# helloybz/CLANE

Hardware: AMD Instinct MI355X
Metric: embedding-update iters/sec (Jacobi sweeps of Z <- X + gamma*P*Z, P frozen) (higher is better)
Workload: dtype f32; 1 GPU; R-MAT |V|=2000000 |E|=40000000 d=256 f32, gamma=0.76, CosineSimilarity (reference mode), seeds 3/4

## Files before the change

clane_amd/_hip.py:

```python
from __future__ import annotations

import abc
import ctypes as C
import os
import threading
from pathlib import Path
from typing import Optional

import torch

LIB_NAME = "libclane_hip.so"
LIB_PATH = Path(__file__).resolve().parent / LIB_NAME
ABI_VERSION = 5

SCORE_REFERENCE, SCORE_PER_EDGE, SCORE_RAW_DOT = 0, 1, 2
SPMM_SINKS_UNTOUCHED = 1
SPMM_TABLE_BEYOND_CACHE = 2
SCORE_FUSE_SOFTMAX = 1
SCORE_MODES = {"reference": SCORE_REFERENCE, "per_edge": SCORE_PER_EDGE, "raw_dot": SCORE_RAW_DOT}

_p, _i64, _i32 = C.c_void_p, C.c_int64, C.c_int32

SIGNATURES = {
    "clane_abi_version": (C.c_int, []),
    "clane_last_error": (C.c_char_p, []),
    "clane_build_info": (C.c_char_p, []),
    "clane_xcc_ids": (C.c_int, [_p, _i64, _i32, _p]),
    "clane_check_csr": (C.c_int, [_p, _p, _i64, _i64, _i64, _p, _p]),
    "clane_spmm_partials_len": (_i64, [_i64, _i64]),
    "clane_reduce_ws_len": (_i64, []),
    "clane_reduce_partials": (C.c_int, [_p, _i64, _p, _p, _p]),
    "clane_spmm_split_slab_len": (_i64, [_i64, _i32]),
    "clane_spmm_class_slab_len": (_i64, [_i64, _i32]),
    "clane_device_alloc": (C.c_int, [_i64, C.POINTER(_p)]),
    "clane_device_alloc_contiguous": (C.c_int, [_i64, C.POINTER(_p)]),
    "clane_device_free": (C.c_int, [_p]),
    "clane_ipc_export": (C.c_int, [_p, _p]),
    "clane_ipc_open": (C.c_int, [_p, C.POINTER(_p)]),
    "clane_ipc_close": (C.c_int, [_p]),
}
IPC_HANDLE_BYTES = 64
for _s in ("f32", "f64", "bf16"):
    SIGNATURES[f"clane_row_sqnorm_{_s}"] = (C.c_int, [_p, _i64, _i32, _i64, _p, _p])
    SIGNATURES[f"clane_edge_score_{_s}"] = (
        C.c_int, [_p, _p, _i64, _i64, _p, _i64, _i32, _i32, _p, _p, _p, _i32, _i64, _p, _i64, _p])
    _g = C.c_double if _s == "f64" else C.c_float
    SIGNATURES[f"clane_spmm_update_{_s}"] = (
        C.c_int, [_p, _p, _p, _i64, _i64, _p, _i64, _p, _i64, _g, _p, _i64, _i32, _i64, _i32, _p, _p, _p])
    SIGNATURES[f"clane_spmm_update_long_{_s}"] = (
        C.c_int, [_p, _p, _p, _p, _i64, _i32, _i64, _p, _i64, _p, _i64, _g, _p, _i64, _i32, _p, _p, _p])
    SIGNATURES[f"clane_spmm_update_split_{_s}"] = (
        C.c_int,
        [_p, _p, _p, _p, _p, _p, _i64, _i64, _i64, _i64, _p, _i64, _p, _i64, _g, _p, _i64, _i32, _p, _p, _p, _p])
    SIGNATURES[f"clane_spmm_update_class_{_s}"] = (
        C.c_int,
        [_p, _p, _p, _p, _p, _i64, _i32, _p, _p, _i64, _i64, _p, _i64, _p, _i64, _g, _p, _i64, _i32, _i32, _p, _p, _p, _p])
    SIGNATURES[f"clane_edge_score_class_{_s}"] = (
        C.c_int, [_p, _p, _p, _p, _p, _p, _i64, _i32, _p, _p, _i64, _i64, _p, _i64, _i32, _i32, _p, _p, _p, _i32, _p, _p])
    SIGNATURES[f"clane_gather_rows_{_s}"] = (C.c_int, [_p, _i64, _p, _i64, _i32, _p, _i64, _p])
    SIGNATURES[f"clane_l1_distance_{_s}"] = (C.c_int, [_p, _i64, _p, _i64, _i64, _i32, _p, _p, _p, _p])
SIGNATURES["clane_spmm_update_owned_f32"] = (
    C.c_int, [_p, _p, _p, _i32, _i64, _p, _i64, _p, _i64, C.c_float, _p, _i64, _i32, _i32, _p, _p])
for _s in ("f32", "f64"):
    SIGNATURES[f"clane_degree_weighted_sums_{_s}"] = (C.c_int, [_p, _p, _p, _i64, _p, _p, _p])
    SIGNATURES[f"clane_edge_score_finalize_{_s}"] = (C.c_int, [_p, _p, _i64, _i64, _i32, _p, _p, _p, _p])
    SIGNATURES[f"clane_segment_softmax_{_s}"] = (C.c_int, [_p, _i64, _p, _i64, _i64, _p, _i64, _p])
    SIGNATURES[f"clane_pair_cosine_{_s}"] = (C.c_int, [_p, _i64, _p, _i64, _i64, _i32, _p, _p, _p])
    SIGNATURES[f"clane_edge_score_pair_{_s}"] = (
        C.c_int, [_p, _p, _i64, _i64, _p, _i64, _p, _i64, _i32, _p, _i32, _i64, _p, _i64, _p])
    SIGNATURES[f"clane_edge_score_class_pair_{_s}"] = (
        C.c_int, [_p, _p, _p, _p, _p, _p, _i64, _i32, _p, _p, _i64, _i64, _p, _i64, _p, _i64, _i32, _p, _i32, _p, _p])
for _s in ("f32", "f64", "bf16"):
    SIGNATURES[f"clane_project_rows_{_s}"] = (C.c_int, [_p, _i64, _i32, _i64, _p, _p, _i64, _p])
    SIGNATURES[f"clane_pair_project_{_s}"] = (C.c_int, [_p, _i64, _i32, _i64, _p, _p, _i64, _p, _p, _p, _p])
    SIGNATURES[f"clane_pair_grad_{_s}"] = (C.c_int, [_p, _i64, _i32, _i64, _p, _p, _i64, _p, _p, _p, _p, _p, _p, _p])
for _s in ("f32", "f64"):
    SIGNATURES[f"clane_pair_loss_{_s}"] = (C.c_int, [_p, _p, _i64, _i32, _p, _p, _p, _p, _p, _p, _p])
    SIGNATURES[f"clane_adam_step_{_s}"] = (C.c_int, [_p, _p, _p, _p, _i64, C.c_double, _p, _p, _p])
SIGNATURES["clane_pair_grad_ws_len"] = (_i64, [_i64, _i32])
RANK_MAX_K = 32
for _s in ("f32", "f64", "bf16"):
    SIGNATURES[f"clane_rank_scores_{_s}"] = (
        C.c_int, [_p, _i64, _p, _i64, _i64, _i32, _p, _i64, _i32, _p, _p, _p, _p, _p, _i32, _i32, _i32, _p, _p, _p])
    SIGNATURES[f"clane_pair_score_{_s}"] = (C.c_int, [_p, _i64, _p, _i64, _i64, _i32, _p, _p, _i64, _i32, _p, _p, _p, _p])
    SIGNATURES[f"clane_rank_count_{_s}"] = (
        C.c_int, [_p, _i64, _p, _i64, _i64, _i32, _p, _p, _i64, _i32, _p, _p, _p, _p, _p, _i32, _i32, _p, _p, _p])
for _s in ("f32", "f64"):
    SIGNATURES[f"clane_rank_merge_{_s}"] = (C.c_int, [_p, _p, _i64, _i32, _i32, _p, _p, _p])
SIGNATURES["clane_pair_labels"] = (C.c_int, [_p, _p, _i64, _p, _p, _i64, _p, _p])
PROBE_MAX_CLASSES = 64
PROBE_WRITE_G, PROBE_WRITE_PRED = 1, 2
PROBE_PRED_TOPK = 4
for _s in ("f32", "f64", "bf16"):
    SIGNATURES[f"clane_probe_forward_{_s}"] = (
        C.c_int, [_p, _i64, _i32, _i64, _p, _p, _i64, _p, _i64, _p, _p, _i32, _i32, _i32, _p, _p, _p, _p, _i64, _p])
    SIGNATURES[f"clane_probe_grad_{_s}"] = (C.c_int, [_p, _i64, _i32, _i64, _p, _i64, _p, _i32, _p, _p, _p, _p])
    SIGNATURES[f"clane_probe_forward_ovr_{_s}"] = (
        C.c_int, [_p, _i64, _i32, _i64, _p, _p, _i64, _p, _i64, _p, _p, _p, _i32, _i32, _i32, _i32, _p, _p, _p, _p, _i64, _p])
SIGNATURES["clane_probe_loss_ws_len"] = (_i64, [_i64, _i32])
SIGNATURES["clane_probe_grad_ws_len"] = (_i64, [_i64, _i32, _i32])
for _s in ("f32", "f64", "bf16"):
    SIGNATURES[f"clane_kmeans_assign_{_s}"] = (
        C.c_int, [_p, _i64, _i32, _i64, _p, _i64, _p, _p, _i32, _i32, _p, _i64, _p, _i64, _p])
    SIGNATURES[f"clane_kmeans_update_{_s}"] = (
        C.c_int, [_p, _i64, _i32, _i64, _p, _p, _i64, _i32, _i32, _p, _p, _p, _p, _p])
SIGNATURES["clane_kmeans_update_ws_len"] = (_i64, [_i64, _i32, _i32, _i32])
for _s in ("f32", "f64", "bf16"):
    _g = C.c_double if _s == "f64" else C.c_float
    SIGNATURES[f"clane_embed_rows_{_s}"] = (
        C.c_int, [_p, _p, _i64, _p, _i64, _p, _i64, _i64, _i32, _i32, _p, _p, _p, _i64, _g, _i32, _i32, _i32, _p, _i64,
                  _p, _p, _p, _p])

PCA_ACCUMULATE = 1
for _s in ("f32", "f64", "bf16"):
    SIGNATURES[f"clane_column_sums_{_s}"] = (C.c_int, [_p, _i64, _i32, _i64, _p, _i64, _i32, _p, _p, _p])
# ... 345 lines not shown
    def probe_forward_ovr(self, Z, d: int, rows, ymask, split, W, bias, col_state, F: int, C: int, max_labels: int,
                          loss_ws, loss, G=None, pred=None, top_k: bool = True):
        raise NotImplementedError(f"{type(self).__name__} has no probe_forward_ovr")

    def probe_grad_ws_len(self, n: int, K: int, d: int) -> int:
        raise NotImplementedError(f"{type(self).__name__} has no probe_grad_ws_len")

    def probe_grad(self, Z, d: int, rows, G, ws, dW, db):
        raise NotImplementedError(f"{type(self).__name__} has no probe_grad")

    def kmeans_assign(self, Z, d: int, rows, centres, csq, assign, best):
        raise NotImplementedError(f"{type(self).__name__} has no kmeans_assign")

    def kmeans_update_ws_len(self, n: int, R: int, K: int, d: int) -> int:
        raise NotImplementedError(f"{type(self).__name__} has no kmeans_update_ws_len")

    def kmeans_update(self, Z, d: int, order, seg, centres_old, ws, centres_new, csq_new):
        raise NotImplementedError(f"{type(self).__name__} has no kmeans_update")

    def column_sums_ws_len(self, n: int, d: int) -> int:
        raise NotImplementedError(f"{type(self).__name__} has no column_sums_ws_len")

    def column_sums(self, Z, d: int, rows, ws, sums, accumulate: bool = False):
        raise NotImplementedError(f"{type(self).__name__} has no column_sums")

    def gram_ws_len(self, n: int, d: int) -> int:
        raise NotImplementedError(f"{type(self).__name__} has no gram_ws_len")

    def gram(self, Z, d: int, rows, mu, ws, G, accumulate: bool = False):
        raise NotImplementedError(f"{type(self).__name__} has no gram")

    def project_affine(self, Z, d: int, rows, mu, W, Y):
        raise NotImplementedError(f"{type(self).__name__} has no project_affine")

    def csr_spmm_segment(self) -> int:
        raise NotImplementedError(f"{type(self).__name__} has no csr_spmm_segment")

    def csr_spmm_ws_len(self, n_rows: int, nnz: int, l: int) -> int:
        raise NotImplementedError(f"{type(self).__name__} has no csr_spmm_ws_len")

    def csr_spmm(self, S, B, l: int, out, a=None, s=None, ws=None):
        raise NotImplementedError(f"{type(self).__name__} has no csr_spmm")

    def csr_row_sums(self, S, sums, ws=None):
        raise NotImplementedError(f"{type(self).__name__} has no csr_row_sums")

    def has_spmm_owned(self, dtype, d: int) -> bool:
        return False

    def make_owned_plan(self, plan: dict, chunk: int, device):
        raise NotImplementedError(f"{type(self).__name__} has no make_owned_plan")

    def spmm_update_owned(self, colidx, P, plan, block_threads: int, row0: int, Z_old, X, gamma: float, Z_new, d: int,
                          partials, beyond_cache: bool = False, loads: int = 0):
        raise NotImplementedError(f"{type(self).__name__} has no spmm_update_owned")

    def bind(self, method: str, *args, **kwargs):
        fn = getattr(self, method)
        return lambda: fn(*args, **kwargs)

    def embed_rows(self, rowptr, colidx, X_new, Z, table_rows: int, d: int, mode: int, sums2, sq, S, gamma: float,
                   tolerence: int, max_rounds: int, Z_out, rounds, delta, P_out=None, flags: int = 0):
        raise NotImplementedError(f"{type(self).__name__} has no embed_rows")


class HipKernels(KernelBackend):

    def __init__(self, lib: Optional[C.CDLL] = None):
        self.lib = lib if lib is not None else load_library()
        self._tls = threading.local()

    def _invoke(self, fn, what: str, *cargs):
        rec = getattr(self._tls, "recording", None)
        if rec is not None:
            rec.append((fn, cargs, what))
        else:
            self._check(fn(*cargs), what)

    def bind(self, method: str, *args, **kwargs):
        self._tls.recording = []
        try:
            getattr(self, method)(*args, **kwargs)
            (fn, cargs, what), = self._tls.recording
        finally:
            self._tls.recording = None
        check = self._check
        return lambda: check(fn(*cargs), what)

    def _check(self, rc: int, what: str):
        if rc != 0:
            raise ClaneHipError(f"{what} failed ({rc}): {self.lib.clane_last_error().decode()}")

    @staticmethod
    def _stream(t: torch.Tensor):
        if not t.is_cuda:
            raise ClaneHipError("HipKernels needs tensors in GPU memory (got a CPU tensor); there is no CPU path")
        return torch.cuda.current_stream(t.device).cuda_stream

    def _fn(self, base: str, dtype: torch.dtype):
        try:
            return getattr(self.lib, f"{base}_{_SUFFIX[dtype]}")
        except KeyError:
            raise TypeError(f"{base}: unsupported dtype {dtype}") from None

    def spmm_partials_len(self, nrows: int, n_long: int) -> int:
        return int(self.lib.clane_spmm_partials_len(nrows, n_long))

    def xcc_ids(self, n_blocks: int, block_threads: int = 256, device=None) -> torch.Tensor:
        out = torch.full((n_blocks,), -1, dtype=torch.int32, device=device if device is not None else "cuda")
        self._check(self.lib.clane_xcc_ids(out.data_ptr(), n_blocks, block_threads, self._stream(out)), "clane_xcc_ids")
        return out

    def check_csr(self, rowptr: torch.Tensor, colidx: torch.Tensor, nrows: int, n_edges: int, table_rows: int) -> None:
        if rowptr.dtype != torch.int64 or colidx.dtype != torch.int32 or rowptr.numel() < nrows + 1 or colidx.numel() < n_edges:
            raise ValueError("check_csr: rowptr must be int64 [nrows + 1], colidx int32 [n_edges]")
        status = torch.zeros(1, dtype=torch.int32, device=rowptr.device)
        self._check(self.lib.clane_check_csr(rowptr.data_ptr(), colidx.data_ptr(), nrows, n_edges, table_rows,
                                             status.data_ptr(), self._stream(rowptr)), "clane_check_csr")
        bad = int(status.item())
# ... 100 lines not shown
        if not (Z_old.dtype == X.dtype == Z_new.dtype):
            raise ValueError("spmm_update_long: Z_old, X, Z_new must share a dtype")
        self._invoke(self._fn("clane_spmm_update_long", Z_old.dtype), "clane_spmm_update_long",
                     _vec(rowptr, torch.int64, "rowptr"), _vec(colidx, torch.int32, "colidx"),
                     _vec(P, acc_dtype(Z_old.dtype), "P"), _vec(long_rows, torch.int32, "long_rows"),
                     long_rows.numel(), waves_per_row, row0, zo, ldz, xp, ldx, gamma, zn, ldo, d,
                     _mirror_arg(mirror, Z_new.dtype), _vec(partials, torch.float64, "partials"), self._stream(Z_old))

    def spmm_split_slab_len(self, n_segments: int, d: int) -> int:
        return int(self.lib.clane_spmm_split_slab_len(n_segments, d))

    def spmm_update_split(self, rowptr, colidx, P, split_rows, seg_ptr, seg_row, edges_per_segment: int, row0: int,
                          Z_old, X, gamma: float, Z_new, d: int, slab, partials, mirror: Optional[Mirror] = None):
        zo, ldz = _mat(Z_old, "Z_old")
        xp, ldx = _mat(X, "X")
        zn, ldo = _mat(Z_new, "Z_new")
        self._invoke(self._fn("clane_spmm_update_split", Z_old.dtype), "clane_spmm_update_split",
                     _vec(rowptr, torch.int64, "rowptr"), _vec(colidx, torch.int32, "colidx"),
                     _vec(P, acc_dtype(Z_old.dtype), "P"), _vec(split_rows, torch.int32, "split_rows"),
                     _vec(seg_ptr, torch.int64, "seg_ptr"), _vec(seg_row, torch.int32, "seg_row"),
                     split_rows.numel(), seg_row.numel(), edges_per_segment, row0, zo, ldz, xp, ldx, gamma, zn, ldo, d,
                     _vec(slab, acc_dtype(Z_old.dtype), "slab"), _mirror_arg(mirror, Z_new.dtype),
                     _vec(partials, torch.float64, "partials"), self._stream(Z_old))

    def spmm_class_slab_len(self, n_slots: int, d: int) -> int:
        return int(self.lib.clane_spmm_class_slab_len(n_slots, d))

    def spmm_update_class(self, colidx, P, item_e0, item_len, item_slot, items_per_block: int, class_rows, slot_ptr,
                          row0: int, Z_old, X, gamma: float, Z_new, d: int, slab, partials,
                          mirror: Optional[Mirror] = None, beyond_cache: bool = False):
        zo, ldz = _mat(Z_old, "Z_old")
        xp, ldx = _mat(X, "X")
        zn, ldo = _mat(Z_new, "Z_new")
        n_items = item_e0.numel()
        if n_items % items_per_block or item_len.numel() != n_items or item_slot.numel() != n_items:
            raise ValueError("spmm_update_class: the item arrays must hold whole blocks of items_per_block items")
        self._invoke(self._fn("clane_spmm_update_class", Z_old.dtype), "clane_spmm_update_class",
                     _vec(colidx, torch.int32, "colidx"), _vec(P, acc_dtype(Z_old.dtype), "P"),
                     _vec(item_e0, torch.int64, "item_e0"), _vec(item_len, torch.int32, "item_len"),
                     _vec(item_slot, torch.int32, "item_slot"), n_items // items_per_block, items_per_block,
                     _vec(class_rows, torch.int32, "class_rows"), _vec(slot_ptr, torch.int64, "slot_ptr"),
                     class_rows.numel(), row0, zo, ldz, xp, ldx, gamma, zn, ldo, d,
                     SPMM_TABLE_BEYOND_CACHE if beyond_cache else 0,
                     _vec(slab, acc_dtype(Z_old.dtype), "slab"), _mirror_arg(mirror, Z_new.dtype),
                     _vec(partials, torch.float64, "partials"), self._stream(Z_old))

    def has_spmm_owned(self, dtype, d: int) -> bool:
        return dtype == torch.float32 and 64 < d <= 256

    def make_owned_plan(self, plan: dict, chunk: int, device) -> OwnedPlan:
        return OwnedPlan(plan, chunk, device)

    def spmm_update_owned(self, colidx, P, plan: OwnedPlan, block_threads: int, row0: int, Z_old, X, gamma: float,
                          Z_new, d: int, partials, beyond_cache: bool = False, loads: int = 0):
        zo, ldz = _mat(Z_old, "Z_old")
        xp, ldx = _mat(X, "X")
        zn, ldo = _mat(Z_new, "Z_new")
        if not (Z_old.dtype == X.dtype == Z_new.dtype == torch.float32):
            raise TypeError("spmm_update_owned: float32 tables only")
        lanes = 32 if d <= 128 else 64
        if plan.max_batch_vrows * lanes * 16 > OWNED_LDS_LIMIT:
            raise ValueError(f"spmm_update_owned: {plan.max_batch_vrows} virtual rows per batch do not fit the LDS")
        if (plan.max_edge > min(colidx.numel(), P.numel()) or plan.max_row >= min(X.shape[0], Z_new.shape[0])
                or row0 + plan.max_row >= Z_old.shape[0] or plan.max_part >= partials.numel()):
            raise ValueError("spmm_update_owned: the plan reaches outside colidx / P, the tables or the partials")
        self._invoke(self.lib.clane_spmm_update_owned_f32, "clane_spmm_update_owned",
                     _vec(colidx, torch.int32, "colidx"), _vec(P, torch.float32, "P"), C.cast(C.pointer(plan.c), _p),
                     int(block_threads), row0, zo, ldz, xp, ldx, gamma, zn, ldo, d,
                     (SPMM_TABLE_BEYOND_CACHE if beyond_cache else 0) | ((int(loads) & 0xff) << 8),
                     _vec(partials, torch.float64, "partials"), self._stream(Z_old))

    def reduce_partials(self, partials, n: int, ws, out):
        self._invoke(self.lib.clane_reduce_partials, "clane_reduce_partials",
                     _vec(partials, torch.float64, "partials"), n, _vec(ws, torch.float64, "ws"),
                     _vec(out, torch.float64, "out"), self._stream(out))

    def l1_distance(self, A, B, d: int, ws, out, sq_a: Optional[torch.Tensor] = None):
        ap, lda = _mat(A, "A")
        bp, ldb = _mat(B, "B")
        self._check(self._fn("clane_l1_distance", A.dtype)(
            ap, lda, bp, ldb, A.shape[0], d, self._sq_arg(sq_a, A.dtype), _vec(ws, torch.float64, "ws"),
            _vec(out, torch.float64, "out"), self._stream(A)), "clane_l1_distance")

    def gather_rows(self, src, idx, d: int, dst):
        sp, lds = _mat(src, "src")
        dp, ldd = _mat(dst, "dst")
        self._invoke(self._fn("clane_gather_rows", src.dtype), "clane_gather_rows",
                     sp, lds, _vec(idx, torch.int32, "idx"), idx.numel(), d, dp, ldd, self._stream(src))

    def project_rows(self, Z, d: int, W, Y):
        zp, ldz = _mat(Z, "Z")
        yp, ldy = _mat(Y, "Y")
        acc = acc_dtype(Z.dtype)
        if tuple(W.shape) != (2 * d, d):
            raise ValueError(f"project_rows: W must be [2d, d] = [{2 * d}, {d}], got {tuple(W.shape)}")
        if Y.dtype != acc or Y.shape[0] < Z.shape[0]:
            raise ValueError(f"project_rows: Y must be {acc} with at least {Z.shape[0]} rows")
        self._check(self._fn("clane_project_rows", Z.dtype)(
            zp, Z.shape[0], d, ldz, _vec(W, acc, "W"), yp, ldy, self._stream(Z)), "clane_project_rows")

    def edge_score_pair(self, rowptr, colidx, nrows: int, row0: int, S, N, d: int, scores, long_threshold: int = 0,
                        long_rows=None, fuse_softmax: bool = False):
        sp, lds = _mat(S, "S")
        np_, ldn = _mat(N, "N")
        if S.dtype != N.dtype:
            raise ValueError("edge_score_pair: S and N must share a dtype")
        n_long = 0 if long_rows is None else long_rows.numel()
        self._check(self._fn("clane_edge_score_pair", S.dtype)(
            _vec(rowptr, torch.int64, "rowptr"), _vec(colidx, torch.int32, "colidx"), nrows, row0, sp, lds, np_, ldn, d,
            _vec(scores, S.dtype, "scores"), SCORE_FUSE_SOFTMAX if fuse_softmax else 0, long_threshold,
            None if n_long == 0 else _vec(long_rows, torch.int32, "long_rows"), n_long,
            self._stream(S)), "clane_edge_score_pair")

    def edge_score_class_pair(self, rowptr, colidx, item_e0, item_len, item_slot, item_row, items_per_block: int,
                              class_rows, slot_ptr, row0: int, S, N, d: int, scores, stats=None,
                              fuse_softmax: bool = False, n_slots: Optional[int] = None, row_parts: int = 1):
        sp, lds = _mat(S, "S")
        np_, ldn = _mat(N, "N")
        if S.dtype != N.dtype:
            raise ValueError("edge_score_class_pair: S and N must share a dtype")
        n_items = item_e0.numel()
        if n_items % items_per_block or any(t.numel() != n_items for t in (item_len, item_slot, item_row)):
            raise ValueError("edge_score_class_pair: the item arrays must hold whole blocks of items_per_block items")
# ... 406 lines not shown
```

clane_amd/csrc/clane_abi.hip:

```cpp
#include "../../include/clane_hip.h"

#include <hip/hip_runtime.h>

#include <climits>
#include <cstdarg>
#include <cstdio>
#include <cstring>

#include "build_p.h"
#include "content_pca.h"
#include "edge_score.h"
#include "device_utils.h"
#include "kmeans.h"
#include "label_probe.h"
#include "multilabel_probe.h"
#include "new_rows.h"
#include "link_eval.h"
#include "link_rank.h"
#include "pair_train.h"
#include "projection.h"
#include "sparse_rows.h"
#include "spmm_update.h"

namespace {
// ... 428 lines not shown
        spmm_class_combine_kernel<T, VEC, LPR>
            <<<unsigned(ceil_div(n_split, kWave / LPR)), kCombineWaves * kWave, 0, (hipStream_t)stream>>>(
            split_rows, seg_ptr, n_split, row0, slab, ld_slab, Z_old, ldz, X, ldx, gamma, Z_new, ldo, d, mir, false, delta_partials);
    });
    return check_launch("spmm_update_split");
}

template <typename T, typename PT>
int spmm_update_class(const int32_t *colidx, const PT *P, const int64_t *item_e0, const int32_t *item_len,
                      const int32_t *item_slot, int64_t n_blocks, int32_t items_per_block, const int32_t *class_rows,
                      const int64_t *slot_ptr, int64_t n_rows, int64_t row0, const T *Z_old, int64_t ldz, const T *X,
                      int64_t ldx, typename Elem<T>::acc_t gamma, T *Z_new, int64_t ldo, int32_t d, int32_t flags,
                      typename Elem<T>::acc_t *slab, const clane_mirror_t *mirror, double *delta_partials,
                      void *stream) {
    REQUIRE(mirror_ok(mirror, d), "spmm_update_class: incomplete mirror descriptor");
    REQUIRE(n_blocks >= 0 && n_blocks <= INT32_MAX && n_rows >= 0 && n_rows <= INT32_MAX && row0 >= 0 && d > 0,
            "spmm_update_class: bad shape");
    REQUIRE(items_per_block >= kWavesPerBlock && items_per_block <= kMaxItemsPerBlock,
            "spmm_update_class: items_per_block must be in [%d, %d]", kWavesPerBlock, kMaxItemsPerBlock);
    REQUIRE(ldz >= d && ldx >= d && ldo >= d, "spmm_update_class: leading dimension < d");
    if (n_rows == 0) return CLANE_OK;
    REQUIRE(colidx && P && item_e0 && item_len && item_slot && class_rows && slot_ptr && Z_old && X && Z_new && slab &&
                delta_partials,
            "spmm_update_class: null pointer");
    REQUIRE((const void *)Z_new != (const void *)Z_old, "spmm_update_class: Z_new must not alias Z_old");
    REQUIRE(aligned16(slab), "spmm_update_class: slab must be 16-byte aligned");
    const Layout L = pick_layout<T>(d, {Z_old, X, Z_new, mirror_alignment_probe(mirror, Z_new)},
                                    {ldz, ldx, ldo, mirror && mirror->row_ptr ? mirror->ld : ldo});
    const int64_t ld_slab = ceil_div(d, 8) * 8;
    const Mirror<T> mir = make_mirror<T>(mirror);
    dispatch_layout<T>(L, [&]<int VEC, int LPR>() {
        constexpr int U = VEC > 1 ? CLANE_LONG_U : 4;
        constexpr int kDeepU = (LPR == 32 && VEC == 4 && sizeof(T) == 4) ? CLANE_CLASS_U32
                               : (LPR == 16 && VEC == 8 && sizeof(T) == 2) ? CLANE_CLASS_U16B : 0;
        if (n_blocks > 0 && kDeepU > 0 && (flags & CLANE_SPMM_TABLE_BEYOND_CACHE))
            spmm_class_chunk_kernel<T, PT, VEC, LPR, (kDeepU > 0 ? kDeepU : U)>
                <<<unsigned(n_blocks), kBlock, 0, (hipStream_t)stream>>>(
                    colidx, P, item_e0, item_len, item_slot, items_per_block, Z_old, ldz, d, slab, ld_slab);
        else if (n_blocks > 0)
            spmm_class_chunk_kernel<T, PT, VEC, LPR, U><<<unsigned(n_blocks), kBlock, 0, (hipStream_t)stream>>>(
                colidx, P, item_e0, item_len, item_slot, items_per_block, Z_old, ldz, d, slab, ld_slab);
        spmm_class_combine_kernel<T, VEC, LPR>
            <<<unsigned(ceil_div(n_rows, kWave / LPR)), kCombineWaves * kWave, 0, (hipStream_t)stream>>>(
            class_rows, slot_ptr, n_rows, row0, slab, ld_slab, Z_old, ldz, X, ldx, gamma, Z_new, ldo, d, mir,
            (flags & CLANE_SPMM_TABLE_BEYOND_CACHE) != 0, delta_partials);
    });
    return check_launch("spmm_update_class");
}

constexpr int64_t kOwnedLdsReserve = 1024;
constexpr int64_t kLdsPerCU = 160 * 1024;
constexpr int64_t kLdsDefaultLimit = 64 * 1024;

template <typename T, typename PT>
int spmm_update_owned(const int32_t *colidx, const PT *P, const clane_owned_plan_t *plan, int32_t block_threads,
                      int64_t row0, const T *Z_old, int64_t ldz, const T *X, int64_t ldx,
                      typename Elem<T>::acc_t gamma, T *Z_new, int64_t ldo, int32_t d, int32_t flags,
                      double *delta_partials, void *stream) {
    using A = typename Elem<T>::acc_t;
    REQUIRE(plan, "spmm_update_owned: null plan");
    REQUIRE(plan->n_groups >= 0 && row0 >= 0 && d > 0, "spmm_update_owned: bad shape");
    REQUIRE(plan->n_steps >= 1 && plan->n_steps <= kOwnedMaxSteps, "spmm_update_owned: n_steps must be in [1, %d]",
            kOwnedMaxSteps);
    REQUIRE(plan->chunk >= kWave && plan->chunk % kWave == 0, "spmm_update_owned: chunk must be a positive multiple of 64");
    REQUIRE(block_threads >= kWave && block_threads <= kOwnedMaxBlock && block_threads % kWave == 0,
            "spmm_update_owned: block_threads must be a multiple of 64 in [64, %d]", kOwnedMaxBlock);
    REQUIRE(ldz >= d && ldx >= d && ldo >= d, "spmm_update_owned: leading dimension < d");
    REQUIRE(plan->max_batch_vrows >= 0, "spmm_update_owned: negative max_batch_vrows");
    if (plan->n_groups == 0) return CLANE_OK;
    REQUIRE(colidx && P && plan->grp_bat_ptr && plan->bat_vrow_ptr && plan->bat_row_ptr && plan->bat_seg_ptr &&
                plan->seg_e0 && plan->seg_len && plan->seg_vrow && plan->row_id && plan->row_part && plan->row_vptr &&
                Z_old && X && Z_new && delta_partials,
            "spmm_update_owned: null pointer");
    REQUIRE((const void *)Z_new != (const void *)Z_old, "spmm_update_owned: Z_new must not alias Z_old");
    const Layout L = pick_layout<T>(d, {Z_old, X, Z_new}, {ldz, ldx, ldo});
    REQUIRE(L.vec && (L.lpr == 32 || L.lpr == 64) && d <= L.lpr * Elem<T>::kVec,
            "spmm_update_owned: no instance for d=%d with these operands (16-byte packs, 17..64 packs per row)", d);
    const int64_t lds = int64_t(plan->max_batch_vrows) * L.lpr * Elem<T>::kVec * int64_t(sizeof(A));
    REQUIRE(lds + kOwnedLdsReserve <= kLdsPerCU, "spmm_update_owned: %lld virtual rows per batch need %lld bytes of LDS",
            (long long)plan->max_batch_vrows, (long long)lds);
    const OwnedPlan op{plan->grp_bat_ptr, plan->bat_vrow_ptr, plan->bat_row_ptr, plan->bat_seg_ptr, plan->seg_e0,
                       plan->seg_len, plan->seg_vrow, plan->row_id, plan->row_part, plan->row_vptr, plan->n_steps,
                       plan->chunk};
    const bool beyond = (flags & CLANE_SPMM_TABLE_BEYOND_CACHE) != 0;
    int rc = CLANE_OK;
    auto launch = [&]<int VEC, int LPR, int U>() {
        auto *kernel = spmm_owned_kernel<T, PT, VEC, LPR, U>;
        if (lds > kLdsDefaultLimit) {
            static int64_t granted = 0;
            if (lds > granted) {
                const hipError_t e = hipFuncSetAttribute(reinterpret_cast<const void *>(kernel),
                                                         hipFuncAttributeMaxDynamicSharedMemorySize, int(lds));
                if (e != hipSuccess) {
                    rc = fail(CLANE_ERR_LAUNCH, "spmm_update_owned: %lld bytes of LDS: %s", (long long)lds,
                              hipGetErrorString(e));
                    return;
                }
                granted = lds;
            }
        }
        kernel<<<unsigned(plan->n_groups), unsigned(block_threads), size_t(lds), (hipStream_t)stream>>>(
            colidx, P, op, row0, Z_old, ldz, X, ldx, gamma, Z_new, ldo, d, beyond, delta_partials);
    };
    constexpr int KV = Elem<T>::kVec;
    const int asked = (flags >> 8) & 0xff;
    REQUIRE(asked == 0 || asked == 8 || asked == 12 || (L.lpr == 32 && asked == 6),
            "spmm_update_owned: no instance with %d row loads in flight", asked);
    const int loads = asked ? asked : (L.lpr == 32 && beyond) ? CLANE_CLASS_U32 : CLANE_LONG_U;
    if (L.lpr == 32) {
        if (loads == 6) launch.template operator()<KV, 32, 6>();
        else if (loads == 12) launch.template operator()<KV, 32, 12>();
        else launch.template operator()<KV, 32, 8>();
    } else {
        if (loads == 12) launch.template operator()<KV, 64, 12>();
        else launch.template operator()<KV, 64, 8>();
    }
    if (rc != CLANE_OK) return rc;
    return check_launch("spmm_update_owned");
}

template <typename T>
int l1_distance(const T *A, int64_t lda, const T *B, int64_t ldb, int64_t nrows, int32_t d,
                typename Elem<T>::acc_t *sq_a, double *ws, double *out, void *stream) {
    REQUIRE(nrows >= 0 && d > 0 && lda >= d && ldb >= d, "l1_distance: bad shape");
    REQUIRE(ws && out, "l1_distance: null workspace/output");
    REQUIRE(nrows == 0 || (A && B), "l1_distance: null pointer");
    const Layout L = pick_layout<T>(d, {A, B}, {lda, ldb});
    if (sq_a != nullptr) {
        const Layout LA = pick_layout<T>(d, {A}, {lda});
        REQUIRE(LA.vec == L.vec && LA.lpr == L.lpr,
                "l1_distance: sq_a needs B as aligned as A (the lane layout of row_sqnorm on A)");
    }
    int grid = 1;
    dispatch_layout<T>(L, [&]<int VEC, int LPR>() {
        grid = grid_for_waves(ceil_div(nrows > 0 ? nrows : 1, (kWave / LPR) * stream_rows(LPR)));
        if (grid > kReduceGrid) grid = kReduceGrid;
        l1_distance_kernel<T, VEC, LPR><<<grid, kBlock, 0, (hipStream_t)stream>>>(A, lda, B, ldb, nrows, d, sq_a, ws);
    });
    reduce_fixed_kernel<<<1, 1024, 0, (hipStream_t)stream>>>(ws, grid, grid, 1, out);
    return check_launch("l1_distance");
}

template <typename T>
int gather_rows(const T *src, int64_t lds, const int32_t *idx, int64_t n, int32_t d, T *dst, int64_t ldd, void *stream) {
    REQUIRE(n >= 0 && d > 0 && lds >= d && ldd >= d, "gather_rows: bad shape");
    if (n == 0) return CLANE_OK;
    REQUIRE(src && idx && dst, "gather_rows: null pointer");
    const Layout L = pick_layout<T>(d, {src, dst}, {lds, ldd});
    dispatch_layout<T>(L, [&]<int VEC, int LPR>() {
        const int grid = grid_for_waves(ceil_div(n, kWave / LPR));
        gather_rows_kernel<T, VEC, LPR><<<grid, kBlock, 0, (hipStream_t)stream>>>(src, lds, idx, n, d, dst, ldd);
    });
    return check_launch("gather_rows");
}

template <typename T>
int pair_cosine(const T *A, int64_t lda, const T *B, int64_t ldb, int64_t nrows, int32_t d,
                typename Elem<T>::acc_t *out, double *ws, void *stream) {
    REQUIRE(nrows >= 0 && d > 0 && lda >= d && ldb >= d, "pair_cosine: bad shape");
    if (nrows == 0) return CLANE_OK;
    REQUIRE(A && B && out && ws, "pair_cosine: null pointer");
    const Layout L = pick_layout<T>(d, {A, B}, {lda, ldb});
    int grid = 1;
    dispatch_layout<T>(L, [&]<int VEC, int LPR>() {
        grid = grid_for_waves(ceil_div(nrows, kWave / LPR));
        if (grid > kReduceGrid) grid = kReduceGrid;
        pair_dot_kernel<T, VEC, LPR><<<grid, kBlock, 0, (hipStream_t)stream>>>(A, lda, B, ldb, nrows, d, out, ws);
    });
    double *sums2 = ws + 2 * kReduceGrid;
    reduce_fixed_kernel<<<1, 1024, 0, (hipStream_t)stream>>>(ws, grid, grid, 2, sums2);
    int sgrid = int(ceil_div(nrows, kBlock));
// ... 688 lines not shown
                                CT *Z_new, int64_t ldo, int32_t d, int64_t long_threshold, int32_t flags,             \
                                const clane_mirror_t *mirror, double *delta_partials, void *stream) {                \
        return spmm_update<T, PT>(rowptr, colidx, P, nrows, row0, reinterpret_cast<const T *>(Z_old), ldz,            \
                                  reinterpret_cast<const T *>(X), ldx, gamma, reinterpret_cast<T *>(Z_new), ldo, d,   \
                                  long_threshold, flags, mirror, delta_partials, stream);                             \
    }                                                                                                                 \
    int clane_spmm_update_long_##SUF(const int64_t *rowptr, const int32_t *colidx, const PT *P,                       \
                                     const int32_t *long_rows, int64_t n_long, int32_t waves_per_row, int64_t row0, const CT *Z_old,         \
                                     int64_t ldz, const CT *X, int64_t ldx, GT gamma, CT *Z_new, int64_t ldo,         \
                                     int32_t d, const clane_mirror_t *mirror, double *delta_partials, void *stream) { \
        return spmm_update_long<T, PT>(rowptr, colidx, P, long_rows, n_long, waves_per_row, row0,                     \
                                       reinterpret_cast<const T *>(Z_old), ldz, reinterpret_cast<const T *>(X), ldx,  \
                                       gamma, reinterpret_cast<T *>(Z_new), ldo, d, mirror, delta_partials, stream);  \
    }
#define CLANE_SPLIT_WRAPPER(SUF, CT, T, PT, GT)                                                                         \
    int clane_spmm_update_split_##SUF(const int64_t *rowptr, const int32_t *colidx, const PT *P,                      \
                                      const int32_t *split_rows, const int64_t *seg_ptr, const int32_t *seg_row,      \
                                      int64_t n_split, int64_t n_segments, int64_t edges_per_segment, int64_t row0,   \
                                      const CT *Z_old, int64_t ldz, const CT *X, int64_t ldx, GT gamma, CT *Z_new,    \
                                      int64_t ldo, int32_t d, GT *slab, const clane_mirror_t *mirror,                 \
                                      double *delta_partials, void *stream) {                                         \
        return spmm_update_split<T, PT>(rowptr, colidx, P, split_rows, seg_ptr, seg_row, n_split, n_segments,         \
                                        edges_per_segment, row0, reinterpret_cast<const T *>(Z_old), ldz,             \
                                        reinterpret_cast<const T *>(X), ldx, gamma, reinterpret_cast<T *>(Z_new),     \
                                        ldo, d, slab, mirror, delta_partials, stream);                                \
    }
CLANE_SPLIT_WRAPPER(f32, float, float, float, float)
CLANE_SPLIT_WRAPPER(f64, double, double, double, double)
CLANE_SPLIT_WRAPPER(bf16, uint16_t, bf16_t, float, float)
#undef CLANE_SPLIT_WRAPPER
#define CLANE_CLASS_WRAPPER(SUF, CT, T, PT, GT)                                                                        \
    int clane_spmm_update_class_##SUF(const int32_t *colidx, const PT *P, const int64_t *item_e0,                     \
                                      const int32_t *item_len, const int32_t *item_slot, int64_t n_blocks,            \
                                      int32_t items_per_block, const int32_t *class_rows, const int64_t *slot_ptr,    \
                                      int64_t n_rows, int64_t row0, const CT *Z_old, int64_t ldz, const CT *X,        \
                                      int64_t ldx, GT gamma, CT *Z_new, int64_t ldo, int32_t d, int32_t flags,        \
                                      GT *slab, const clane_mirror_t *mirror, double *delta_partials, void *stream) { \
        return spmm_update_class<T, PT>(colidx, P, item_e0, item_len, item_slot, n_blocks, items_per_block,           \
                                        class_rows, slot_ptr, n_rows, row0, reinterpret_cast<const T *>(Z_old), ldz,  \
                                        reinterpret_cast<const T *>(X), ldx, gamma, reinterpret_cast<T *>(Z_new),     \
                                        ldo, d, flags, slab, mirror, delta_partials, stream);                         \
    }
CLANE_CLASS_WRAPPER(f32, float, float, float, float)
CLANE_CLASS_WRAPPER(f64, double, double, double, double)
CLANE_CLASS_WRAPPER(bf16, uint16_t, bf16_t, float, float)
#undef CLANE_CLASS_WRAPPER
int clane_spmm_update_owned_f32(const int32_t *colidx, const float *P, const clane_owned_plan_t *plan,
                                int32_t block_threads, int64_t row0, const float *Z_old, int64_t ldz, const float *X,
                                int64_t ldx, float gamma, float *Z_new, int64_t ldo, int32_t d, int32_t flags,
                                double *delta_partials, void *stream) {
    return spmm_update_owned<float, float>(colidx, P, plan, block_threads, row0, Z_old, ldz, X, ldx, gamma, Z_new, ldo,
                                           d, flags, delta_partials, stream);
}
int64_t clane_spmm_class_slab_len(int64_t n_slots, int32_t d) { return n_slots * (ceil_div(d, 8) * 8); }
int64_t clane_spmm_split_slab_len(int64_t n_segments, int32_t d) { return n_segments * (ceil_div(d, 8) * 8); }

CLANE_SPMM_WRAPPERS(f32, float, float, float, float)
CLANE_SPMM_WRAPPERS(f64, double, double, double, double)
CLANE_SPMM_WRAPPERS(bf16, uint16_t, bf16_t, float, float)
#undef CLANE_SPMM_WRAPPERS

int clane_reduce_partials(const double *partials, int64_t n, double *ws, double *out, void *stream) {
    if (n < 0 || !out || !ws || (n > 0 && !partials))
        return fail(CLANE_ERR_INVALID_ARGUMENT, "reduce_partials: bad arguments");
    if (n <= 8192) {
        reduce_fixed_kernel<<<1, 1024, 0, (hipStream_t)stream>>>(partials, n, n, 1, out);
    } else {
        const int64_t slice = ceil_div(n, kReduceGrid);
        const int grid = int(ceil_div(n, slice));
        reduce_slices_kernel<<<grid, kBlock, 0, (hipStream_t)stream>>>(partials, n, slice, ws);
        reduce_fixed_kernel<<<1, 1024, 0, (hipStream_t)stream>>>(ws, grid, grid, 1, out);
    }
    return check_launch("reduce_partials");
}

int clane_l1_distance_f32(const float *A, int64_t lda, const float *B, int64_t ldb, int64_t nrows, int32_t d,
                          float *sq_a, double *ws, double *out, void *stream) {
    return l1_distance<float>(A, lda, B, ldb, nrows, d, sq_a, ws, out, stream);
}
int clane_l1_distance_f64(const double *A, int64_t lda, const double *B, int64_t ldb, int64_t nrows, int32_t d,
                          double *sq_a, double *ws, double *out, void *stream) {
    return l1_distance<double>(A, lda, B, ldb, nrows, d, sq_a, ws, out, stream);
}
int clane_l1_distance_bf16(const uint16_t *A, int64_t lda, const uint16_t *B, int64_t ldb, int64_t nrows, int32_t d,
                           float *sq_a, double *ws, double *out, void *stream) {
    return l1_distance<bf16_t>(reinterpret_cast<const bf16_t *>(A), lda, reinterpret_cast<const bf16_t *>(B), ldb,
                               nrows, d, sq_a, ws, out, stream);
}

int clane_gather_rows_f32(const float *src, int64_t lds, const int32_t *idx, int64_t n, int32_t d, float *dst,
                          int64_t ldd, void *stream) {
    return gather_rows<float>(src, lds, idx, n, d, dst, ldd, stream);
}
int clane_gather_rows_f64(const double *src, int64_t lds, const int32_t *idx, int64_t n, int32_t d, double *dst,
                          int64_t ldd, void *stream) {
    return gather_rows<double>(src, lds, idx, n, d, dst, ldd, stream);
}
int clane_gather_rows_bf16(const uint16_t *src, int64_t lds, const int32_t *idx, int64_t n, int32_t d, uint16_t *dst,
                           int64_t ldd, void *stream) {
    return gather_rows<bf16_t>(reinterpret_cast<const bf16_t *>(src), lds, idx, n, d,
                               reinterpret_cast<bf16_t *>(dst), ldd, stream);
}

int clane_pair_cosine_f32(const float *A, int64_t lda, const float *B, int64_t ldb, int64_t nrows, int32_t d,
                          float *out, double *ws, void *stream) {
    return pair_cosine<float>(A, lda, B, ldb, nrows, d, out, ws, stream);
// ... 197 lines not shown
```

clane_amd/csrc/spmm_update.h:

```cpp
#pragma once

#include "device_utils.h"

#ifndef CLANE_SPMM_U
#define CLANE_SPMM_U 8
#endif
#ifndef CLANE_SPMM_DYNAMIC
#define CLANE_SPMM_DYNAMIC 1
#endif
#ifndef CLANE_COMBINE_WAVES
#define CLANE_COMBINE_WAVES 2
#endif
#ifndef CLANE_SPMM_PREFETCH
#define CLANE_SPMM_PREFETCH 1
#endif
#ifndef CLANE_SPMM_MIN_WAVES
#define CLANE_SPMM_MIN_WAVES 0
#endif

namespace clane {

template <typename A>
struct EdgeChunk {
    int c;
// ... 114 lines not shown
    return rsum;
}

template <typename T, int VEC, int GROUP>
__device__ __forceinline__ void mirror_store(const Mirror<T> &mirror, int64_t row, int col, const Pack<T, VEC> &out,
                                             bool writer, int group_lane, int base) {
    if (mirror.row_ptr == nullptr) return;
    const int64_t s0 = mirror.row_ptr[row], s1 = mirror.row_ptr[row + 1];
    for (int64_t s = s0; s < s1; s += GROUP) {
        const int n = s1 - s < GROUP ? int(s1 - s) : GROUP;
        int32_t mine = 0;
        if (group_lane < n) mine = mirror.slot[s + group_lane];
        for (int j = 0; j < n; ++j) {
            int32_t place;
            if constexpr (GROUP == kWave) place = lane_get_uniform(mine, j);
            else place = lane_get(mine, base + j);
            if (writer) store_pack<T, VEC>(mirror.row(place) + col, out);
        }
    }
}

template <typename T, int VEC, int GROUP>
__device__ __forceinline__ void mirror_store_prefetched(const Mirror<T> &mirror, int64_t m0, int64_t m1, int32_t mine,
                                                        int col, const Pack<T, VEC> &out, bool writer, int group_lane,
                                                        int base) {
    if (mirror.row_ptr == nullptr) return;
    const int n = m1 - m0 < GROUP ? int(m1 - m0) : GROUP;
    for (int j = 0; j < n; ++j) {
        int32_t place;
        if constexpr (GROUP == kWave) place = lane_get_uniform(mine, j);
        else place = lane_get(mine, base + j);
        if (writer) store_pack<T, VEC>(mirror.row(place) + col, out);
    }
    for (int64_t s = m0 + GROUP; s < m1; s += GROUP) {
        const int k = m1 - s < GROUP ? int(m1 - s) : GROUP;
        int32_t more = 0;
        if (group_lane < k) more = mirror.slot[s + group_lane];
        for (int j = 0; j < k; ++j) {
            int32_t place;
            if constexpr (GROUP == kWave) place = lane_get_uniform(more, j);
            else place = lane_get(more, base + j);
            if (writer) store_pack<T, VEC>(mirror.row(place) + col, out);
        }
    }
}

#if CLANE_SPMM_MIN_WAVES > 0
#define CLANE_SPMM_BOUNDS __launch_bounds__(kBlock, CLANE_SPMM_MIN_WAVES)
#else
#define CLANE_SPMM_BOUNDS __launch_bounds__(kBlock)
#endif

template <typename T, typename PT, int VEC, int LPR, int U, bool MIRRORED>
__global__ CLANE_SPMM_BOUNDS void spmm_update_kernel(
    const int64_t *__restrict__ rowptr, const int32_t *__restrict__ colidx, const PT *__restrict__ P, int64_t nrows,
    int64_t row0, const T *__restrict__ Zold, int64_t ldz, const T *__restrict__ X, int64_t ldx,
    typename Elem<T>::acc_t gamma, T *__restrict__ Znew, int64_t ldo, int d, int64_t long_threshold,
    bool skip_sinks, int rows_per_block, Mirror<T> mirror, bool nt_store, double *__restrict__ partials) {
    using A = typename Elem<T>::acc_t;
    __shared__ int64_t s_rowptr[kMaxRowsPerBlock + 1];
    __shared__ int64_t s_mptr[MIRRORED ? kMaxRowsPerBlock + 1 : 1];
    __shared__ double s_rowsum[kMaxRowsPerBlock];
    __shared__ int s_next;
    __shared__ int s_done;

    const int lane = lane_id();
    const int wave = __builtin_amdgcn_readfirstlane(threadIdx.x / kWave);
    const int sub = lane / LPR;
    const int sl = lane % LPR;
    const int64_t row_begin = int64_t(blockIdx.x) * rows_per_block;
    const int nb = int((row_begin + rows_per_block < nrows ? row_begin + rows_per_block : nrows) - row_begin);

    for (int i = threadIdx.x; i <= nb; i += kBlock) {
        s_rowptr[i] = rowptr[row_begin + i];
        if constexpr (MIRRORED) s_mptr[i] = mirror.row_ptr[row_begin + i];
    }
    for (int i = threadIdx.x; i < nb; i += kBlock) s_rowsum[i] = 0.0;
    if (threadIdx.x == 0) {
        s_next = kWavesPerBlock;
        s_done = 0;
    }
    __syncthreads();
    auto places_of = [&]([[maybe_unused]] int row, [[maybe_unused]] int64_t &m0, [[maybe_unused]] int64_t &m1) -> int32_t {
        if constexpr (MIRRORED) {
            m0 = s_mptr[row];
            m1 = s_mptr[row + 1];
            return lane < m1 - m0 ? mirror.slot[m0 + lane] : 0;
        } else {
            return 0;
        }
    };

    auto claim = [&]([[maybe_unused]] int prev) -> int {
#if CLANE_SPMM_DYNAMIC
        int v = 0;
        if (lane == 0) v = atomicAdd(&s_next, 1);
        return __builtin_amdgcn_readfirstlane(v);
#else
        return prev + kWavesPerBlock;
#endif
    };

    int cur = wave;
    int64_t e0 = 0, e1 = 0, m0 = 0, m1 = 0;
    int32_t places = 0;
    EdgeChunk<A> ch{0, A(0)};
    if (cur < nb) {
        e0 = s_rowptr[cur];
        e1 = s_rowptr[cur + 1];
        ch = load_chunk<A, PT>(colidx, P, e0, e1);
        places = places_of(cur, m0, m1);
    }
    while (cur < nb) {
        const int nxt = claim(cur);
        int64_t n0 = 0, n1 = 0, mn0 = 0, mn1 = 0;
        int32_t places_n = 0;
        EdgeChunk<A> chn{0, A(0)};
        if (nxt < nb) {
            n0 = s_rowptr[nxt];
            n1 = s_rowptr[nxt + 1];
#if CLANE_SPMM_PREFETCH
            chn = load_chunk<A, PT>(colidx, P, n0, n1);
#endif
            places_n = places_of(nxt, mn0, mn1);
        }
        if (!(long_threshold > 0 && e1 - e0 > long_threshold) && !(skip_sinks && e1 == e0)) {
            const int64_t r = row_begin + cur;
            A rsum = A(0);
            for (int t0 = 0; t0 < d; t0 += LPR * VEC) {
                const int c0 = t0 + sl * VEC;
                const bool col_ok = c0 < d;
                const bool writer = col_ok && sub == 0;
                Pack<T, VEC> x{}, zo{};
                if (writer) {
                    x = load_pack_stream<T, VEC>(X + r * ldx + c0);
                    zo = load_pack_stream<T, VEC>(Zold + (row0 + r) * ldz + c0);
                }
                A acc[VEC];
#pragma unroll
                for (int k = 0; k < VEC; ++k) acc[k] = A(0);
                gather_accumulate<T, PT, VEC, LPR, U>(colidx, P, e0, e1, Zold + (col_ok ? c0 : 0), ldz, col_ok, acc, ch, true);
                fold_subwaves<LPR>(acc);
                Pack<T, VEC> out{};
                if (writer) rsum += finish_pack<T, VEC>(x, zo, acc, gamma, e1 > e0, Znew + r * ldo + c0, out, nt_store);
                if constexpr (MIRRORED)
                    mirror_store_prefetched<T, VEC, kWave>(mirror, m0, m1, places, c0, out, writer, lane, 0);
            }
            rsum = group_sum<kWave>(rsum);
            if (lane == 0) s_rowsum[cur] = double(rsum);
        }
        cur = nxt;
        e0 = n0;
        e1 = n1;
        m0 = mn0;
        m1 = mn1;
        places = places_n;
#if CLANE_SPMM_PREFETCH
        ch = chn;
#else
        if (cur < nb) ch = load_chunk<A, PT>(colidx, P, e0, e1);
#endif
    }
    if (!last_wave_of_block(&s_done)) return;
    double dsum = 0.0;
    for (int i = lane; i < nb; i += kWave) dsum += s_rowsum[i];
    dsum = group_sum<kWave>(dsum);
    if (lane == 0) partials[blockIdx.x] = dsum;
}

#ifndef CLANE_SUBROW_MIN_WAVES
#define CLANE_SUBROW_MIN_WAVES 0
#endif
#if CLANE_SUBROW_MIN_WAVES > 0
#define CLANE_SUBROW_BOUNDS __launch_bounds__(kBlock, (sizeof(typename Elem<T>::acc_t) == 8 ? 1 : CLANE_SUBROW_MIN_WAVES))
#else
#define CLANE_SUBROW_BOUNDS __launch_bounds__(kBlock)
#endif
template <typename T, typename PT, int VEC, int LPR, int U, bool MIRRORED>
__global__ CLANE_SUBROW_BOUNDS void spmm_update_subrow_kernel(
    const int64_t *__restrict__ rowptr, const int32_t *__restrict__ colidx, const PT *__restrict__ P, int64_t nrows,
    int64_t row0, const T *__restrict__ Zold, int64_t ldz, const T *__restrict__ X, int64_t ldx,
    typename Elem<T>::acc_t gamma, T *__restrict__ Znew, int64_t ldo, int d, int64_t long_threshold,
    bool skip_sinks, int rows_per_block, Mirror<T> mirror, bool nt_store, double *__restrict__ partials) {
    using A = typename Elem<T>::acc_t;
    static_assert(LPR < kWave, "use spmm_update_kernel for rows that fill a wave");
    static_assert(LPR % U == 0, "a sub-wave's edge buffer is consumed in whole groups of U");
    __shared__ int64_t s_rowptr[kMaxRowsPerBlock + 1];
    __shared__ int64_t s_mptr[MIRRORED ? kMaxRowsPerBlock + 1 : 1];
    __shared__ double s_rowsum[kMaxRowsPerBlock];
    __shared__ int s_next;
    __shared__ int s_done;

    const int lane = lane_id();
    const int sub = lane / LPR;
    const int sl = lane % LPR;
    const int sub_base = sub * LPR;
    const int64_t row_begin = int64_t(blockIdx.x) * rows_per_block;
    const int nb = int((row_begin + rows_per_block < nrows ? row_begin + rows_per_block : nrows) - row_begin);
    const int c0 = sl * VEC;
    const bool col_ok = c0 < d;
    const int c0s = col_ok ? c0 : 0;

    for (int i = threadIdx.x; i <= nb; i += kBlock) {
        s_rowptr[i] = rowptr[row_begin + i];
        if constexpr (MIRRORED) s_mptr[i] = mirror.row_ptr[row_begin + i];
    }
    for (int i = threadIdx.x; i < nb; i += kBlock) s_rowsum[i] = 0.0;
    if (threadIdx.x == 0) {
        s_next = 0;
        s_done = 0;
    }
    __syncthreads();

    int mine = 0;
    bool have = false;
    bool done = false;
    int64_t e_next = 0;
    int64_t e_end = 0;
    int nbuf = 0, pos = 0;
    int c = 0;
    A p = A(0);
    [[maybe_unused]] int64_t m0 = 0, m1 = 0;
    [[maybe_unused]] int32_t places = 0;
    Pack<T, VEC> x{}, zo{};
    A acc[VEC];
#pragma unroll
    for (int k = 0; k < VEC; ++k) acc[k] = A(0);

    for (;;) {
        if (pos >= nbuf && !done) {
            if (e_next == e_end) {
                if (have) {
                    const int64_t r = row_begin + mine;
                    A rsum = A(0);
                    Pack<T, VEC> out{};
                    if (col_ok) rsum = finish_pack<T, VEC>(x, zo, acc, gamma, true, Znew + r * ldo + c0, out, nt_store);
                    if constexpr (MIRRORED)
                        mirror_store_prefetched<T, VEC, LPR>(mirror, m0, m1, places, c0, out, col_ok, sl, sub_base);
                    rsum = group_sum<LPR>(rsum);
                    if (sl == 0) s_rowsum[mine] = double(rsum);
                    have = false;
                }
                for (;;) {
                    int v = 0;
                    if (sl == 0) v = atomicAdd(&s_next, 1);
                    mine = lane_get(v, sub_base);
                    if (mine >= nb) {
                        done = true;
                        break;
                    }
// ... 12 lines not shown
                        m0 = s_mptr[mine];
                        m1 = s_mptr[mine + 1];
                        places = sl < m1 - m0 ? mirror.slot[m0 + sl] : 0;
                    }
                    if (col_ok) {
                        x = load_pack_stream<T, VEC>(X + r * ldx + c0);
                        zo = load_pack_stream<T, VEC>(Zold + (row0 + r) * ldz + c0);
                    }
#pragma unroll
                    for (int k = 0; k < VEC; ++k) acc[k] = A(0);
                    have = true;
                    break;
                }
            }
            pos = 0;
            nbuf = 0;
            c = 0;
            p = A(0);
            if (!done) {
                const int64_t left = e_end - e_next;
                nbuf = left < LPR ? int(left) : LPR;
                if (sl < nbuf) {
                    c = colidx[e_next + sl];
                    p = A(P[e_next + sl]);
                }
                e_next += nbuf;
            }
        }
        if (__all(done)) break;
        Pack<T, VEC> z[U];
        A pj[U];
#pragma unroll
        for (int u = 0; u < U; ++u) {
            const int src = sub_base + ((pos + u) & (LPR - 1));
            const int cj = lane_get(c, src);
            pj[u] = lane_get(p, src);
            z[u] = load_pack<T, VEC>(Zold + int64_t(cj) * ldz + c0s);
        }
#pragma unroll
        for (int u = 0; u < U; ++u) {
#pragma unroll
            for (int k = 0; k < VEC; ++k) {
                A zv = Elem<T>::to_acc(z[u].v[k]);
                zv = pj[u] != A(0) ? zv : A(0);
                acc[k] = fma(pj[u], zv, acc[k]);
            }
        }
        pos += U;
    }
    if (!last_wave_of_block(&s_done)) return;
    double dsum = 0.0;
    for (int i = lane; i < nb; i += kWave) dsum += s_rowsum[i];
    dsum = group_sum<kWave>(dsum);
    if (lane == 0) partials[blockIdx.x] = dsum;
}

template <typename T, typename PT, int VEC, int LPR, int U, int WAVES>
__global__ __launch_bounds__(WAVES *kWave) void spmm_long_kernel(
    const int64_t *__restrict__ rowptr, const int32_t *__restrict__ colidx, const PT *__restrict__ P,
    const int32_t *__restrict__ long_rows, int64_t row0, const T *__restrict__ Zold, int64_t ldz,
    const T *__restrict__ X, int64_t ldx, typename Elem<T>::acc_t gamma, T *__restrict__ Znew, int64_t ldo, int d,
    Mirror<T> mirror, double *__restrict__ partials) {
    using A = typename Elem<T>::acc_t;
    __shared__ A red[WAVES][kWave][VEC];
    const int lane = lane_id();
    const int wave = __builtin_amdgcn_readfirstlane(threadIdx.x / kWave);
    const int sub = lane / LPR;
    const int sl = lane % LPR;
    const int64_t r = long_rows[blockIdx.x];
    const int64_t e0 = rowptr[r];
    const int64_t e1 = rowptr[r + 1];
    const int64_t seg = ceil_div(ceil_div(e1 - e0, WAVES), kWave) * kWave;
    const int active = e1 > e0 ? int(ceil_div(e1 - e0, seg)) : 1;
    if (idle_wave_may_exit(wave < active)) return;
    const int64_t a = e0 + wave * seg;
    const int64_t b = a + seg < e1 ? a + seg : e1;
    const EdgeChunk<A> none{0, A(0)};
    A rsum = A(0);

    for (int t0 = 0; t0 < d; t0 += LPR * VEC) {
        const int c0 = t0 + sl * VEC;
        const bool col_ok = c0 < d;
        const bool writer = wave == 0 && col_ok && sub == 0;
        Pack<T, VEC> x{}, zo{};
        if (writer) {
            x = load_pack_stream<T, VEC>(X + r * ldx + c0);
            zo = load_pack_stream<T, VEC>(Zold + (row0 + r) * ldz + c0);
        }
        A acc[VEC];
#pragma unroll
        for (int k = 0; k < VEC; ++k) acc[k] = A(0);
        gather_accumulate<T, PT, VEC, LPR, U>(colidx, P, a, b, Zold + (col_ok ? c0 : 0), ldz, col_ok, acc, none, false);
        fold_subwaves<LPR>(acc);
        if (wave > 0) {
#pragma unroll
            for (int k = 0; k < VEC; ++k) red[wave][lane][k] = acc[k];
        }
        __syncthreads();
        if (wave == 0) {
            Pack<T, VEC> out{};
            if (writer) {
                for (int w = 1; w < active; ++w) {
#pragma unroll
                    for (int k = 0; k < VEC; ++k) acc[k] += red[w][lane][k];
                }
                rsum += finish_pack<T, VEC>(x, zo, acc, gamma, e1 > e0, Znew + r * ldo + c0, out, false);
            }
// ... 42 lines not shown
        for (int k = 0; k < VEC; ++k) acc[k] = A(0);
        gather_accumulate<T, PT, VEC, LPR, U>(colidx, P, a, b, Zold + (col_ok ? c0 : 0), ldz, col_ok, acc, none, false);
        fold_subwaves<LPR>(acc);
        if (wave > 0) {
#pragma unroll
            for (int k = 0; k < VEC; ++k) red[wave][lane][k] = acc[k];
        }
        __syncthreads();
        if (wave == 0 && col_ok && sub == 0) {
            for (int w = 1; w < active; ++w) {
#pragma unroll
                for (int k = 0; k < VEC; ++k) acc[k] += red[w][lane][k];
            }
            Pack<A, VEC> o;
#pragma unroll
            for (int k = 0; k < VEC; ++k) o.v[k] = acc[k];
            store_pack<A, VEC>(slab + s * ld_slab + c0, o);
        }
        if (t0 + LPR * VEC < d) __syncthreads();
    }
}

}

namespace clane {


#ifndef CLANE_NT_SLAB
#define CLANE_NT_SLAB 1
#endif
template <typename A, int VEC>
__device__ __forceinline__ void slab_store(A *p, const Pack<A, VEC> &v) {
    if constexpr ((CLANE_NT_SLAB & 1) && sizeof(Pack<A, VEC>) == 16) {
        clane_u32x4 w;
        __builtin_memcpy(&w, &v, 16);
        __builtin_nontemporal_store(w, reinterpret_cast<clane_u32x4 *>(p));
    } else {
        store_pack<A, VEC>(p, v);
    }
}
template <typename A, int VEC>
__device__ __forceinline__ Pack<A, VEC> slab_load(const A *p) {
    if constexpr ((CLANE_NT_SLAB & 2) && sizeof(Pack<A, VEC>) == 16) {
        const clane_u32x4 v = __builtin_nontemporal_load(reinterpret_cast<const clane_u32x4 *>(p));
        Pack<A, VEC> out;
        __builtin_memcpy(&out, &v, 16);
        return out;
    } else {
        return load_pack<A, VEC>(p);
    }
}

template <typename T, typename PT, int VEC, int LPR, int U>
__global__ __launch_bounds__(kBlock) void spmm_class_chunk_kernel(
    const int32_t *__restrict__ colidx, const PT *__restrict__ P, const int64_t *__restrict__ item_e0,
    const int32_t *__restrict__ item_len, const int32_t *__restrict__ item_slot, int items_per_block,
    const T *__restrict__ Zold, int64_t ldz, int d, typename Elem<T>::acc_t *__restrict__ slab, int64_t ld_slab) {
    using A = typename Elem<T>::acc_t;
    __shared__ int64_t s_e0[kMaxItemsPerBlock];
    __shared__ int s_len[kMaxItemsPerBlock];
    __shared__ int s_slot[kMaxItemsPerBlock];
    __shared__ int s_next;
    const int lane = lane_id();
    const int wave = __builtin_amdgcn_readfirstlane(threadIdx.x / kWave);
    const int sub = lane / LPR;
    const int sl = lane % LPR;
    const int64_t base = int64_t(blockIdx.x) * items_per_block;
    for (int i = threadIdx.x; i < items_per_block; i += kBlock) {
        s_e0[i] = item_e0[base + i];
        s_len[i] = item_len[base + i];
        s_slot[i] = item_slot[base + i];
    }
    if (threadIdx.x == 0) s_next = kWavesPerBlock;
    __syncthreads();

    auto claim = [&]() -> int {
        int v = 0;
        if (lane == 0) v = atomicAdd(&s_next, 1);
        return __builtin_amdgcn_readfirstlane(v);
    };
    int cur = wave;
    int64_t e0 = 0, e1 = 0;
    EdgeChunk<A> ch{0, A(0)};
    if (cur < items_per_block) {
        e0 = s_e0[cur];
        e1 = e0 + s_len[cur];
        ch = load_chunk<A, PT>(colidx, P, e0, e1);
    }
    while (cur < items_per_block) {
        const int nxt = claim();
        int64_t n0 = 0, n1 = 0;
        EdgeChunk<A> chn{0, A(0)};
        if (nxt < items_per_block) {
            n0 = s_e0[nxt];
            n1 = n0 + s_len[nxt];
            chn = load_chunk<A, PT>(colidx, P, n0, n1);
        }
        if (e1 > e0) {
            A *out = slab + int64_t(s_slot[cur]) * ld_slab;
            for (int t0 = 0; t0 < d; t0 += LPR * VEC) {
                const int c0 = t0 + sl * VEC;
                const bool col_ok = c0 < d;
                A acc[VEC];
#pragma unroll
                for (int k = 0; k < VEC; ++k) acc[k] = A(0);
                gather_accumulate<T, PT, VEC, LPR, U>(colidx, P, e0, e1, Zold + (col_ok ? c0 : 0), ldz, col_ok, acc, ch, true);
                fold_subwaves<LPR>(acc);
                if (col_ok && sub == 0) {
                    Pack<A, VEC> o;
#pragma unroll
                    for (int k = 0; k < VEC; ++k) o.v[k] = acc[k];
                    slab_store<A, VEC>(out + c0, o);
                }
            }
        }
        cur = nxt;
        e0 = n0;
        e1 = n1;
        ch = chn;
    }
}

constexpr int kCombineWaves = CLANE_COMBINE_WAVES;
#ifndef CLANE_COMBINE_LOADS
#define CLANE_COMBINE_LOADS 16
#endif
constexpr int kCombineLoads = CLANE_COMBINE_LOADS;

template <typename T, int VEC, int LPR>
__global__ __launch_bounds__(kCombineWaves *kWave) void spmm_class_combine_kernel(
    const int32_t *__restrict__ class_rows, const int64_t *__restrict__ slot_ptr, int64_t n_rows, int64_t row0,
    const typename Elem<T>::acc_t *__restrict__ slab, int64_t ld_slab, const T *__restrict__ Zold, int64_t ldz,
    const T *__restrict__ X, int64_t ldx, typename Elem<T>::acc_t gamma, T *__restrict__ Znew, int64_t ldo, int d,
    Mirror<T> mirror, bool nt_store, double *__restrict__ partials) {
    using A = typename Elem<T>::acc_t;
    constexpr int kRows = kWave / LPR;
    __shared__ A s_part[kCombineWaves > 1 ? kCombineWaves - 1 : 1][kWave][VEC];
    const int lane = lane_id();
    const int wave = __builtin_amdgcn_readfirstlane(threadIdx.x / kWave);
    const int sub = lane / LPR, sl = lane % LPR;
    const int64_t i = int64_t(blockIdx.x) * kRows + sub;
    const bool live = i < n_rows;
    const int64_t r = live ? class_rows[i] : 0;
    const int64_t s0 = live ? slot_ptr[i] : 0, s1 = live ? slot_ptr[i + 1] : 0;
    const int64_t share = ceil_div(s1 - s0, int64_t(kCombineWaves));
    const int64_t a = s0 + wave * share < s1 ? s0 + wave * share : s1;
    const int64_t b = a + share < s1 ? a + share : s1;
    A rsum = A(0);
    for (int t0 = 0; t0 < d; t0 += LPR * VEC) {
        const int c0 = t0 + sl * VEC;
        const bool ok = live && c0 < d;
        A acc[VEC];
#pragma unroll
        for (int k = 0; k < VEC; ++k) acc[k] = A(0);
        if (ok) {
            int64_t s = a;
            for (; s + kCombineLoads <= b; s += kCombineLoads) {
                Pack<A, VEC> part[kCombineLoads];
#pragma unroll
                for (int u = 0; u < kCombineLoads; ++u) part[u] = slab_load<A, VEC>(slab + (s + u) * ld_slab + c0);
#pragma unroll
                for (int u = 0; u < kCombineLoads; ++u) {
#pragma unroll
                    for (int k = 0; k < VEC; ++k) acc[k] += part[u].v[k];
                }
            }
#pragma unroll 4
            for (; s < b; ++s) {
                const Pack<A, VEC> part = slab_load<A, VEC>(slab + s * ld_slab + c0);
#pragma unroll
                for (int k = 0; k < VEC; ++k) acc[k] += part.v[k];
            }
        }
        if constexpr (kCombineWaves > 1) {
            if (t0 > 0) __syncthreads();
            if (wave > 0) {
#pragma unroll
                for (int k = 0; k < VEC; ++k) s_part[wave - 1][lane][k] = acc[k];
            }
            __syncthreads();
        }
        if (wave == 0) {
            Pack<T, VEC> out{};
            if (ok) {
                if constexpr (kCombineWaves > 1) {
#pragma unroll
                    for (int w = 1; w < kCombineWaves; ++w) {
#pragma unroll
                        for (int k = 0; k < VEC; ++k) acc[k] += s_part[w - 1][lane][k];
                    }
                }
                const Pack<T, VEC> x = load_pack_stream<T, VEC>(X + r * ldx + c0);
                const Pack<T, VEC> zo = load_pack_stream<T, VEC>(Zold + (row0 + r) * ldz + c0);
                rsum += finish_pack<T, VEC>(x, zo, acc, gamma, true, Znew + r * ldo + c0, out, nt_store);
            }
            if (live) mirror_store<T, VEC, LPR>(mirror, r, c0, out, ok, sl, sub * LPR);
        }
    }
    if (wave == 0) {
        rsum = group_sum<LPR>(rsum);
        if (live && sl == 0) partials[i] = double(rsum);
    }
}

constexpr int kOwnedMaxSteps = 64;
constexpr int kOwnedMaxBlock = 1024;

struct OwnedPlan {
    const int32_t *grp_bat_ptr;
    const int32_t *bat_vrow_ptr;
    const int32_t *bat_row_ptr;
    const int32_t *bat_seg_ptr;
    const int64_t *seg_e0;
    const int32_t *seg_len;
    const int32_t *seg_vrow;
    const int32_t *row_id;
    const int32_t *row_part;
    const int32_t *row_vptr;
    int n_steps;
    int chunk;
};

template <typename T, typename PT, int VEC, int LPR, int U>
__global__ __launch_bounds__(kOwnedMaxBlock) void spmm_owned_kernel(
    const int32_t *__restrict__ colidx, const PT *__restrict__ P, OwnedPlan plan, int64_t row0,
    const T *__restrict__ Zold, int64_t ldz, const T *__restrict__ X, int64_t ldx, typename Elem<T>::acc_t gamma,
    T *__restrict__ Znew, int64_t ldo, int d, bool nt_store, double *__restrict__ partials) {
    using A = typename Elem<T>::acc_t;
    constexpr int W = LPR * VEC;
    constexpr int kRows = kWave / LPR;
    extern __shared__ __align__(16) unsigned char s_owned_raw[];
    A *s_sum = reinterpret_cast<A *>(s_owned_raw);
    __shared__ int s_cnt[kOwnedMaxSteps];

    const int lane = lane_id();
    const int wave = __builtin_amdgcn_readfirstlane(threadIdx.x / kWave);
    const int nwaves = int(blockDim.x) / kWave;
    const int sub = lane / LPR, sl = lane % LPR;
    const int c0 = sl * VEC;
    const bool col_ok = c0 < d;
    const T *zcol = Zold + (col_ok ? c0 : 0);
    const int n_steps = plan.n_steps;
    const int64_t chunk = plan.chunk;
    const int b0 = plan.grp_bat_ptr[blockIdx.x], b1 = plan.grp_bat_ptr[blockIdx.x + 1];

    for (int b = b0; b < b1; ++b) {
        const int v0 = plan.bat_vrow_ptr[b];
        const int nv = plan.bat_vrow_ptr[b + 1] - v0;
        for (int i = threadIdx.x; i < nv * W; i += int(blockDim.x)) s_sum[i] = A(0);
        if (int(threadIdx.x) < n_steps) s_cnt[threadIdx.x] = 0;
        __syncthreads();
        for (int s = 0; s < n_steps; ++s) {
            const int sa = plan.bat_seg_ptr[b * n_steps + s];
            const int n = plan.bat_seg_ptr[b * n_steps + s + 1] - sa;
            auto claim = [&]() -> int {
                int v = 0;
                if (lane == 0) v = atomicAdd(&s_cnt[s], 1);
                return __builtin_amdgcn_readfirstlane(v);
            };
            int cur = claim();
            int64_t e0 = 0, e1 = 0;
            int vr = 0;
            EdgeChunk<A> ch{0, A(0)};
            if (cur < n) {
                e0 = plan.seg_e0[sa + cur];
                e1 = e0 + plan.seg_len[sa + cur];
                vr = plan.seg_vrow[sa + cur];
                ch = load_chunk<A, PT>(colidx, P, e0, e0 + chunk < e1 ? e0 + chunk : e1);
            }
            while (cur < n) {
                const int nxt = claim();
                int64_t n0 = 0, n1 = 0;
                int vn = 0;
                EdgeChunk<A> chn{0, A(0)};
                if (nxt < n) {
                    n0 = plan.seg_e0[sa + nxt];
                    n1 = n0 + plan.seg_len[sa + nxt];
                    vn = plan.seg_vrow[sa + nxt];
                    chn = load_chunk<A, PT>(colidx, P, n0, n0 + chunk < n1 ? n0 + chunk : n1);
                }
                A *sum = s_sum + vr * W + c0;
                for (int64_t p = e0; p < e1; p += chunk) {
                    const int64_t pe = p + chunk < e1 ? p + chunk : e1;
                    A acc[VEC];
#pragma unroll
                    for (int k = 0; k < VEC; ++k) acc[k] = A(0);
                    gather_accumulate<T, PT, VEC, LPR, U>(colidx, P, p, pe, zcol, ldz, col_ok, acc, ch, p == e0);
                    fold_subwaves<LPR>(acc);
                    if (col_ok && sub == 0) {
                        Pack<A, VEC> t = load_pack<A, VEC>(sum);
#pragma unroll
                        for (int k = 0; k < VEC; ++k) t.v[k] += acc[k];
                        store_pack<A, VEC>(sum, t);
                    }
                }
                cur = nxt;
                e0 = n0;
                e1 = n1;
                vr = vn;
                ch = chn;
            }
            __syncthreads();
        }
        const int r0 = plan.bat_row_ptr[b];
        const int nr = plan.bat_row_ptr[b + 1] - r0;
        for (int j0 = wave * kRows; j0 < nr; j0 += nwaves * kRows) {
            const int j = j0 + sub;
            const bool live = j < nr;
            const bool ok = live && col_ok;
            A rsum = A(0);
            if (ok) {
                const int64_t r = plan.row_id[r0 + j];
                const Pack<T, VEC> x = load_pack_stream<T, VEC>(X + r * ldx + c0);
                const Pack<T, VEC> zo = load_pack_stream<T, VEC>(Zold + (row0 + r) * ldz + c0);
                const int va = plan.row_vptr[r0 + j] - v0, vb = plan.row_vptr[r0 + j + 1] - v0;
                A acc[VEC];
                const Pack<A, VEC> first = load_pack<A, VEC>(s_sum + va * W + c0);
#pragma unroll
                for (int k = 0; k < VEC; ++k) acc[k] = first.v[k];
                for (int v = va + 1; v < vb; ++v) {
                    const Pack<A, VEC> t = load_pack<A, VEC>(s_sum + v * W + c0);
#pragma unroll
                    for (int k = 0; k < VEC; ++k) acc[k] += t.v[k];
                }
                Pack<T, VEC> out{};
                rsum = finish_pack<T, VEC>(x, zo, acc, gamma, true, Znew + r * ldo + c0, out, nt_store);
            }
            rsum = group_sum<LPR>(rsum);
            if (live && sl == 0) partials[plan.row_part[r0 + j]] = double(rsum);
        }
        __syncthreads();
    }
}

}
```

clane_amd/diagnostics.py:

```python
from __future__ import annotations

import numpy as np

from .plan import lanes_per_row


class DiagnosticsMixin:

    def kernel_times_ms(self):
        t = np.array([(e0.elapsed_time(e4), e4.elapsed_time(e1), e1.elapsed_time(e2), e2.elapsed_time(e3))
                      for _, e0, e1, e2, e3, e4 in self.kernel_events]).reshape(-1, 4)
        self.kernel_events = []
        if not len(t):
            return {}
        per_sweep = t.reshape(-1, len(self.blocks), 4).sum(1).mean(0)
        return dict(zip(("split", "hub", "mid", "main"), per_sweep.tolist()))

    def collective_times_ms(self):
        ev, self.collective_events = self.collective_events, []
        if not ev:
            return {}
        t = np.array([(a.elapsed_time(b), b.elapsed_time(c)) for a, b, c in ev])
        return {"exchange_exposed": float(t[:, 0].mean()), "allreduce": float(t[:, 1].mean()), "sweeps_timed": len(ev)}

    def kernel_bytes(self):
        s, ps = self.Zcur.element_size(), self.P.element_size()
        deg = np.diff(self.local.rowptr)
        per_row = deg * (self.d * s + 4 + ps) + np.where(deg > 0, 3 * self.d * s, 0) + 8
        is_long = deg > self.long_threshold if self.long_threshold > 0 else np.zeros_like(deg, dtype=bool)
        is_class = deg > self.class_threshold if self.class_threshold > 0 else np.zeros_like(deg, dtype=bool)
        is_long = is_long | is_class
        is_split = (is_long & (deg > self.split_edges) if self.split_edges > 0 else np.zeros_like(is_long)) & ~is_class
        is_hub = is_long & (deg > self.hub_threshold) & ~is_split & ~is_class
        return {"main": int(per_row[~is_long].sum()) + 8,
                "mid": int(per_row[is_long & ~is_hub & ~is_split & ~is_class].sum()),
                "hub": int(per_row[is_hub].sum()), "split": int(per_row[is_split | is_class].sum())}

    def launches_per_sweep(self) -> int:
        return len(self.blocks) * len(self.tiles)

    def kernel_names(self):
        narrow = self.d > 0 and lanes_per_row(self.d_plan if len(self.tiles) > 1 else self.d, self.dtype) < 64
        return {"main": "spmm_update_subrow_kernel" if narrow else "spmm_update_kernel",
                "mid": "spmm_long_kernel<4 waves>", "hub": "spmm_long_kernel<16 waves>",
                "split": ("spmm_owned_kernel+spmm_class_chunk_kernel+combine" if getattr(self, "class_owned", False)
                          else "spmm_class_chunk_kernel+combine") if self.class_threshold > 0
                else "spmm_split_segment_kernel+combine"}

    def estimated_sweep_seconds(self) -> float:
        s = self.Zcur.element_size()
        d = self.d_full
        total = self.E_total * (d * s + 8) + self.V * 3 * d * s
        return total / max(self.world, 1) / 8e12

    def kernel_config(self) -> dict:
        return {"build": self.k.build_info(), "dtype": str(self.dtype).replace("torch.", ""), "d": self.d,
                "lanes_per_row": lanes_per_row(self.d, self.dtype) if self.d > 0 else 0,
                "rows": int(self.part.n_local), "edges": int(self.E_loc), "launch_blocks": len(self.blocks),
                "long_threshold": self.long_threshold, "score_threshold": self.score_threshold,
                "hub_threshold": self.hub_threshold,
                "split_edges": self.split_edges, "segment_edges": self.segment_edges,
                "class_threshold": self.class_threshold, "class_chunk": self.class_chunk, "class_k1": self.class_k1,
                "class_phases": self.class_phases, "phase_threshold": self.phase_threshold,
                "class_of_row": "xor-fold of 3-bit groups" if self.class_threshold else None,
                "class_affinity": self.class_affinity, "mega_segment_edges": self.mega_segment_edges,
                "class_items_per_block": [c.items_per_block for c in self.class_rows if c is not None][:1],
                "column_tiles": len(self.tiles),
                "fewer_loads_in_flight": bool(self.beyond_cache and self.d > 0 and (str(self.dtype), lanes_per_row(
                    self.d_plan if len(self.tiles) > 1 else self.d, self.dtype)) in (("torch.float32", 32), ("torch.bfloat16", 16))),
                "hot_rows_first": self.hot_rows_first, "exchange": self.exchange,
                **({"class_owned": {"max_edges": self.owned_max_edges, "row_edges": self.owned_row_edges,
                                    "groups": self.owned_groups, "block_threads": self.owned_block_threads,
                                    "batch_vrows": self.owned_batch_vrows, "chunk": self.owned_chunk,
                                    "loads": self.owned_loads}}
                   if getattr(self, "class_owned", False) else {}),
                }

    def exchange_bytes_per_sweep(self) -> int:
        s = self.Zcur.element_size()
        if self.halo:
            return self.part.recv_rows_per_sweep() * self.ld * s
        if self.columns:
            return 0
        return sum((b.span[1] - b.span[0] - b.nrows) * self.ld * s for b in self.blocks if b.span is not None)
```

clane_amd/engine.py:

```python
from __future__ import annotations

import contextlib
import itertools
import threading
from typing import List, Optional

import numpy as np
import torch

from . import _hip, owned, xcd
from .blocks import BlockRows, ClassItems, PartialLayout, SplitRows
from .comm import TorchComm
from .diagnostics import DiagnosticsMixin
from .halo import build_halo_layout
from .partition import Block, HostCSR, LocalCSR, RowPartition, localize
from .plan import (HEAVY_ROW_EDGES, HUB_FACTOR, INFINITY_CACHE_BYTES, L2_BYTES_ALL_XCDS,
                   LONG_THRESHOLD_BY_ROWS_PER_WAVE, MIN_HOT_READ_SHARE, MIN_SEGMENT_EDGES, MIN_SLICE_ROW_BYTES,
                   SOFTMAX_EDGES_PER_WORKGROUP, SPLIT_EDGES, TARGET_SEGMENTS, UNSKEWED_LONG_THRESHOLD, _round_up,
                   column_slice, hot_read_share, lanes_per_row, pick_exchange)
from .staging import StagedZ, StagingMixin, place_piece
from .xcd import (CLASS_CHUNK, CLASS_THRESHOLD_BY_ROWS_PER_WAVE, PHASE_THRESHOLD, PHASES_BY_ROWS_PER_WAVE,
                  class_items)

class SweepEngine(StagingMixin, DiagnosticsMixin):
    STAGE_SLOTS = 3
    N_TABLES = 3
    MAX_TIMED_SWEEPS = 32

    EXCHANGES = ("auto", "columns", "halo", "halo_p2p", "allgather", "allgather_all")

    def __init__(self, csr: HostCSR, X: torch.Tensor, device, kernels=None, *, cosine_mode: str = "reference",
                 process_group=None, chunks: Optional[int] = None, long_threshold: Optional[int] = None,
                 hub_threshold: Optional[int] = None, shuffle: Optional[bool] = None, seed: int = 0,
                 exchange: str = "auto", comm=None, hot_rows_first: bool = True, split_hubs: bool = True,
                 overlap_chunks: bool = True, fused_pack: bool = True, class_threshold: Optional[int] = None,
                 class_chunk: int = CLASS_CHUNK, class_k1: bool = True, class_phases: Optional[int] = None,
                 phase_threshold: int = PHASE_THRESHOLD, delta_stream: bool = False, table_skew=None,
                 table_alloc: str = "torch", column_tiles: Optional[int] = None, class_owned: Optional[bool] = None,
                 owned_max_edges: int = xcd.OWNED_MAX_EDGES, owned_row_edges: int = xcd.OWNED_ROW_EDGES,
                 owned_groups: int = xcd.OWNED_GROUPS, owned_lds_bytes: int = xcd.OWNED_LDS_BYTES,
                 owned_block_threads: int = xcd.OWNED_BLOCK_THREADS, owned_chunk: Optional[int] = None,
                 owned_loads: int = xcd.OWNED_LOADS):
        if X.dim() != 2 or X.shape[0] != csr.num_vertices:
            raise ValueError(f"X must be [V, d] with V={csr.num_vertices}, got {tuple(X.shape)}")
        if cosine_mode not in ("reference", "per_edge"):
            raise ValueError(f"cosine_mode must be 'reference' or 'per_edge', got {cosine_mode!r}")
        csr.validate()
        csr.indeg(device)
        self.k = kernels if kernels is not None else _hip.kernels()
        self.device = torch.device(device)
        self.dtype = X.dtype
        self.acc_dtype = _hip.acc_dtype(X.dtype)
        self.cosine_mode = cosine_mode
        self.table_skew = table_skew
        if table_alloc not in ("torch", "contiguous"):
            raise ValueError("table_alloc must be 'torch' or 'contiguous'")
        self.table_alloc, self._own_tables, self.table_alloc_note = table_alloc, [], None
        self._column_tiles_asked = column_tiles
        X = self._choose_division(csr, X, process_group, comm, exchange)
        self._choose_class_pass(csr, class_threshold, class_chunk, class_k1, class_phases, phase_threshold)
        self._choose_owned(class_owned, owned_max_edges, owned_row_edges, owned_groups, owned_lds_bytes,
                           owned_block_threads, owned_chunk)
        self.owned_loads = int(owned_loads)
        self._build_layout(csr, chunks, shuffle, seed, hot_rows_first)
        self._choose_row_bins(long_threshold, hub_threshold)
        deg = self._upload_structure()
        self._bin_rows(deg, split_hubs)
        self._setup_exchange(deg, fused_pack)
        self._alloc_tables(X, deg)
        self._alloc_scratch(delta_stream, overlap_chunks)
        self._Y = None

    def _choose_division(self, csr: HostCSR, X: torch.Tensor, process_group, comm, exchange: str) -> torch.Tensor:
        self.pg = process_group
        self.comm = comm if comm is not None else (TorchComm(process_group) if process_group is not None else None)
        self.world = self.comm.world if self.comm is not None else 1
        rank = self.comm.rank if self.comm is not None else 0
        if exchange not in self.EXCHANGES:
            raise ValueError("exchange must be 'auto', 'columns', 'halo', 'halo_p2p', 'allgather' or "
                             f"'allgather_all', got {exchange!r}")
        self._forced = self.world == 1 and self.comm is not None and bool(self.comm.force) and exchange in (
            "columns", "allgather", "allgather_all")
        divided = self.world > 1 or self._forced
        if exchange == "auto":
            exchange = pick_exchange(int(X.shape[1]), X.dtype, self.world)
        self._exchange_asked = exchange
        self.exchange = exchange if divided else "none"
        self.columns = divided and exchange == "columns"
        self.C = self.world if self.columns else 1
        self.c = rank if self.columns else 0
        self.V, self.d_full = csr.num_vertices, int(X.shape[1])
        self.E_total = csr.num_edges
        self.col0, self.col1 = column_slice(self.d_full, X.dtype, self.C, self.c) if self.columns else (0, self.d_full)
        if self.columns:
            X = X[:, self.col0:self.col1]
            self.ld_max = _round_up(column_slice(self.d_full, X.dtype, self.C, 0)[1], _hip.VEC_ELEMS[X.dtype])
        self.d = self.col1 - self.col0
        self.ld = _round_up(self.d, _hip.VEC_ELEMS[X.dtype])
        self.row_world, self.row_rank = (1, 0) if self.columns else (self.world, rank)
        self.halo = self.row_world > 1 and exchange in ("halo", "halo_p2p")
        self.p2p = self.halo and exchange == "halo_p2p"
        if self.p2p and self.world > 8:
            raise ValueError("halo_p2p addresses at most 8 GPUs (one box)")
        self.d_plan = self.d
        if self.columns:
            c0, c1 = column_slice(self.d_full, X.dtype, self.C, 0)
            self.d_plan = c1 - c0
        T = self._pick_tiles(csr, X.dtype) if not divided else 1
        cuts = [column_slice(self.d, X.dtype, T, t) for t in range(T)] if self.d > 0 else [(0, 0)]
        self.tiles = [c for c in cuts if c[1] > c[0]] or [(0, self.d)]
        if len(self.tiles) > 1:
            self.d_plan = max(c1 - c0 for c0, c1 in self.tiles)
        self.beyond_cache = csr.num_vertices * self.ld * torch.empty(0, dtype=X.dtype).element_size() > 2 * INFINITY_CACHE_BYTES
        self.ld_plan = _round_up(self.d_plan, _hip.VEC_ELEMS[X.dtype])
        self.rows_per_wave = 64 // lanes_per_row(self.d_plan, X.dtype) if self.d_plan > 0 else 1
        return X

    def _pick_tiles(self, csr: HostCSR, dtype: torch.dtype) -> int:
        asked = self._column_tiles_asked
        if asked is not None:
            if asked < 1:
                raise ValueError("column_tiles must be >= 1")
            return int(asked)
        if dtype != torch.float32 or self.d < 256 or self.d % 128:
            return 1
        if csr.num_vertices * self.ld * 4 <= 2 * INFINITY_CACHE_BYTES:
            return 1
        return min(8, self.d // 128) if hot_read_share(csr, 512) >= MIN_HOT_READ_SHARE else 1

    def _choose_class_pass(self, csr: HostCSR, class_threshold, class_chunk, class_k1, class_phases,
                           phase_threshold) -> None:
        row_bytes = self.ld_plan * torch.empty(0, dtype=self.dtype).element_size()
        self.hot_read_share = hot_read_share(csr, row_bytes) if self.d_plan > 0 else 1.0
        self.class_affinity = True
        if class_threshold is None:
            class_threshold = CLASS_THRESHOLD_BY_ROWS_PER_WAVE[self.rows_per_wave]
            if self.rows_per_wave == 2 and csr.num_vertices * row_bytes <= INFINITY_CACHE_BYTES:
                class_threshold = max(class_threshold, 128)
            if self.hot_read_share < MIN_HOT_READ_SHARE:
                class_threshold = max(class_threshold, HEAVY_ROW_EDGES)
                self.class_affinity = False
        self.class_threshold = int(class_threshold)
        self.class_chunk = int(class_chunk)
        self.class_k1 = bool(class_k1) and self.class_threshold > 0
        if class_phases is None:
            class_phases = (xcd.PHASES_UNDER_COLUMN_TILES if len(self.tiles) > 1 else 0) or \
                PHASES_BY_ROWS_PER_WAVE[self.rows_per_wave]
        self.class_phases = int(class_phases)
        if self.class_threshold == 0 or self.class_phases < 1:
            self.class_phases = 1
        if self.class_phases & (self.class_phases - 1) or self.class_phases > 8:
            raise ValueError("class_phases must be 1, 2, 4 or 8")
        self.phase_threshold = max(int(phase_threshold), self.class_threshold) if self.class_phases > 1 else 0
        if self.class_threshold and not (64 <= self.class_chunk <= 4096 and self.class_chunk % 64 == 0):
            raise ValueError("class_chunk must be a multiple of 64 in [64, 4096]")
        self.mega_segment_edges = int(L2_BYTES_ALL_XCDS // 8 // max(row_bytes, 1)) if self.d_plan > 0 else 0

    def _choose_owned(self, class_owned, max_edges, row_edges, groups, lds_bytes, block_threads, chunk) -> None:
        can = owned.possible(self)
        want = (xcd.OWNED_DEFAULT and self.beyond_cache and self.class_affinity) if class_owned is None else bool(class_owned)
        self.class_owned, self.owned_possible = bool(want and can), bool(can)
        self._lds_bytes = int(lds_bytes)
        self.owned_max_edges, self.owned_row_edges = int(max_edges), int(row_edges)
        self.owned_groups, self.owned_block_threads = int(groups), int(block_threads)
        self.owned_chunk = int(chunk) if chunk is not None else self.class_chunk
        if self.class_owned:
            self._check_owned_settings()

    def _check_owned_settings(self) -> None:
        widths = [c1 - c0 for c0, c1 in self.tiles]
        if self.owned_groups < 1 or self.owned_row_edges < 64 or not (
                64 <= self.owned_block_threads <= 1024 and self.owned_block_threads % 64 == 0):
            raise ValueError("owned_groups must be >= 1, owned_row_edges >= 64, owned_block_threads a multiple of 64 "
                             "in [64, 1024]")
        if not (64 <= self.owned_chunk <= 4096 and self.owned_chunk % 64 == 0):
            raise ValueError("owned_chunk must be a multiple of 64 in [64, 4096]")
        sum_bytes = 16 * lanes_per_row(max(widths), self.dtype)
        self.owned_batch_vrows = self._lds_bytes // sum_bytes
        if self.owned_batch_vrows < 1 or self.owned_batch_vrows * sum_bytes > _hip.OWNED_LDS_LIMIT:
            raise ValueError(f"owned_lds_bytes must hold one sum of {sum_bytes} bytes and stay within "
                             f"{_hip.OWNED_LDS_LIMIT}")

    def _build_layout(self, csr: HostCSR, chunks, shuffle, seed: int, hot_rows_first: bool) -> None:
        if chunks is None:
            chunks = 1 if self.row_world == 1 else 4
        self.hot_rows_first = bool(hot_rows_first)
        if self.halo:
            self.part = build_halo_layout(csr, self.row_world, self.row_rank, chunks, shuffle=shuffle is not False, seed=seed,
                                          hot_rows_first=hot_rows_first, class_threshold=self.class_threshold,
                                          phase_threshold=self.phase_threshold, phases=self.class_phases)
            self.blocks: List[Block] = self.part.blocks
            self.local: LocalCSR = self.part.local
        else:
            live = csr.live_mask() if (self.row_world > 1 and self._exchange_asked == "allgather") else None
            hot = csr.indeg() if (self.row_world == 1 and hot_rows_first and not shuffle) else None
            self.part = RowPartition.create(self.V, self.row_world, self.row_rank, chunks, live_mask=live, shuffle=shuffle,
                                            seed=seed, priority=hot)
            self.blocks = self.part.blocks(spans_for_one_rank=self._forced and not self.columns)
            self.local = localize(csr, self.part, self.device, class_threshold=self.class_threshold,
                                  phase_threshold=self.phase_threshold, phases=self.class_phases)
        if self.part.padded_vertices >= 2 ** 31:
            raise ValueError(f"{self.part.padded_vertices} table rows: column indices are 32-bit (ABI v1); divide the "
                             "rows over more GPUs (exchange='halo') or wait for 64-bit indices")

    def _choose_row_bins(self, long_threshold, hub_threshold) -> None:
        if long_threshold is None:
            long_threshold = LONG_THRESHOLD_BY_ROWS_PER_WAVE[self.rows_per_wave]
            if self.rows_per_wave == 1 and self.class_threshold and self.class_affinity:
                long_threshold = max(long_threshold, self.class_threshold)
            elif self.rows_per_wave == 1 and not self.class_affinity:
                long_threshold = max(long_threshold, UNSKEWED_LONG_THRESHOLD)
            if self.rows_per_wave > 1:
                by_size = 1 << max(7, int(self.local.colidx.shape[0] // 32768).bit_length() - 1)
                long_threshold = min(long_threshold, by_size)
        self.score_threshold = int(long_threshold)
        self.k1_threshold = (min(self.score_threshold, self.class_threshold) if self.score_threshold > 0
                             else self.class_threshold) if self.class_k1 else self.score_threshold
        if self.class_threshold:
            long_threshold = min(long_threshold, self.class_threshold) if long_threshold > 0 else self.class_threshold
        self.long_threshold = int(long_threshold)
# ... 17 lines not shown

    def _bin_rows(self, deg: np.ndarray, split_hubs: bool) -> None:
        dev = self.device
        self.block_rows: List[BlockRows] = []
        self.split_edges = SPLIT_EDGES if split_hubs else 0
        hub_edges = int(deg[deg > SPLIT_EDGES].sum()) // max(1, len(self.blocks))
        self.segment_edges = int(min(SPLIT_EDGES, max(MIN_SEGMENT_EDGES, hub_edges // TARGET_SEGMENTS // 1024 * 1024)))
        max_segments = max_slots = 0
        to_dev = lambda a: torch.from_numpy(a.astype(np.int32)).to(dev) if a.size else None
        for b in self.blocks:
            db = deg[b.local_start:b.local_start + b.nrows]
            is_long = db > self.long_threshold if self.long_threshold > 0 else np.zeros_like(db, dtype=bool)
            is_class = db > self.class_threshold if self.class_threshold > 0 else np.zeros_like(db, dtype=bool)
            is_long = is_long | is_class
            is_split = (is_long & (db > self.split_edges) if self.split_edges > 0 else np.zeros_like(is_long)) & ~is_class
            is_hub = is_long & (db > self.hub_threshold) & ~is_split & ~is_class
            is_mid = is_long & ~is_hub & ~is_split & ~is_class
            k1_long = (db > self.k1_threshold) & ~(is_class if self.class_k1 else np.zeros_like(is_class)) \
                if self.k1_threshold > 0 else np.zeros_like(is_class)
            rows_c, rows_s = np.nonzero(is_class)[0], np.nonzero(is_split)[0]
            layout = PartialLayout.of(row_pass=self.k.spmm_partials_len(b.nrows, 0), n_mid=int(is_mid.sum()),
                                      n_hub=int(is_hub.sum()), n_split=rows_s.size, n_class=rows_c.size,
                                      length=self.k.spmm_partials_len(b.nrows, int(is_long.sum())))
            rows = BlockRows(long=to_dev(np.nonzero(db > self.score_threshold)[0] if self.score_threshold > 0
                                         else np.empty(0, dtype=np.int64)),
                             k1_long=to_dev(np.nonzero(k1_long)[0]), mid=to_dev(np.nonzero(is_mid)[0]),
                             hub=to_dev(np.nonzero(is_hub)[0]), partials=layout)
            if rows_c.size:
                rows_abs = rows_c + b.local_start
                phased = dict(phase_threshold=self.phase_threshold, phases=self.class_phases,
                              mega_segment_edges=self.mega_segment_edges,
                              mega_min_edges=self.part.padded_vertices // 4)
                segments = xcd.row_segments(self.local.rowptr, self.local.colidx, rows_abs, self.colidx,
                                            self.phase_threshold, self.class_phases)
                items = class_items(self.local.rowptr, self.local.colidx, rows_abs, self.class_chunk, None,
                                    row_ids=rows_c, colidx_dev=self.colidx, segments=segments, **phased)
                if self.owned_possible:
                    rows.owned_inputs = (rows_c, rows_abs, segments, phased)
                if self.class_owned:
                    rows.owned = owned.plan_block(self, layout, *rows.owned_inputs)
                rows.klass, rows.n_slots = ClassItems.upload(items, rows_c, dev), int(items["slot_ptr"][-1])
                max_slots = max(max_slots, rows.n_slots)
            if rows_s.size:
                nseg = -(-db[rows_s] // self.segment_edges)
                seg_ptr = np.zeros(rows_s.size + 1, dtype=np.int64)
                np.cumsum(nseg, out=seg_ptr[1:])
                seg_row = np.repeat(np.arange(rows_s.size, dtype=np.int32), nseg)
                rows.split = SplitRows(to_dev(rows_s), torch.from_numpy(seg_ptr).to(dev), torch.from_numpy(seg_row).to(dev))
                max_segments = max(max_segments, int(seg_ptr[-1]))
            self.block_rows.append(rows)
        self.partials = torch.zeros(self.partial_off[-1] * len(self.tiles), dtype=torch.float64, device=dev)
        slab_len = max(1, self.k.spmm_split_slab_len(max_segments, max(self.d_plan, 1)))
        if max_slots:
            slab_len = max(slab_len, self.k.spmm_class_slab_len(max_slots, max(self.d_plan, 1)), 2 * max_slots)
        self.slabs = [torch.zeros(slab_len, dtype=self.acc_dtype, device=dev)
                      for _ in range(2 if len(self.blocks) > 1 else 1)]

    def _per_block(name):
        return property(lambda self: [getattr(r, name) for r in self.block_rows])

    long_rows, k1_long_rows = _per_block("long"), _per_block("k1_long")
    mid_rows, hub_rows, split_rows = _per_block("mid"), _per_block("hub"), _per_block("split")
    class_rows, class_slots, owned_rows = _per_block("klass"), _per_block("n_slots"), _per_block("owned")
    del _per_block

    @property
    def partial_off(self) -> List[int]:
        return list(itertools.accumulate((r.partials.end for r in self.block_rows), initial=0))

    def set_owned(self, on: bool, **settings) -> None:
        if on and not self.owned_possible:
            raise ValueError("this engine has no owned pass: one GPU, fp32, rows or tiles of 65..256 elements")
        if self.device.type == "cuda":
            torch.cuda.synchronize(self.device)
        for name, value in settings.items():
            if name == "lds_bytes":
                self._lds_bytes = int(value)
            elif name in ("max_edges", "row_edges", "groups", "block_threads", "chunk", "loads"):
                setattr(self, "owned_" + name, int(value))
            else:
                raise TypeError(f"set_owned: unknown setting {name!r}")
        self.class_owned = bool(on)
        if on:
            self._check_owned_settings()
        for r in self.block_rows:
            r.owned = owned.plan_block(self, r.partials, *r.owned_inputs) if on and r.owned_inputs is not None else None
        self._plans = {}

    def _setup_exchange(self, deg: np.ndarray, fused_pack: bool) -> None:
        dev = self.device
        self.send_rows: List[Optional[torch.Tensor]] = []
        self.send_buf: List[Optional[torch.Tensor]] = []
        self.mirrors: List[Optional[object]] = []
        self.fused_pack = bool(fused_pack)
        for b in self.blocks:
            ex = b.exchange
            has = ex is not None and ex.send_rows.size > 0 and not self.p2p
            self.send_rows.append(torch.from_numpy(ex.send_rows).to(dev) if has else None)
            self.send_buf.append(torch.zeros(ex.send_rows.size, self.ld, dtype=self.dtype, device=dev) if has
                                 else (torch.zeros(0, self.ld, dtype=self.dtype, device=dev) if ex is not None else None))
            mirror = None
            if has and self.fused_pack:
                rel = ex.send_rows.astype(np.int64) - b.local_start
                if rel.min() < 0 or rel.max() >= b.nrows or (deg[ex.send_rows] == 0).any():
                    raise AssertionError("halo send list holds a row outside its chunk or a row that never changes")
                row_ptr = np.zeros(b.nrows + 1, dtype=np.int64)
                np.cumsum(np.bincount(rel, minlength=b.nrows), out=row_ptr[1:])
# ... 238 lines not shown
                self.P.zero_()
            self._all_reduce(self.P)
            for b, rows in zip(self.blocks, self.block_rows):
                rp = self.rowptr[b.local_start:]
                k.edge_score_finalize(rp, self.colidx, b.nrows, b.row0, mode, self.sums2, sq, self.P)
                k.segment_softmax(rp, b.nrows, self.P, 0, self.score_threshold if rows.long is not None else 0,
                                  rows.long)
        self.P_valid = True

    def build_P_bilinear(self, W: torch.Tensor) -> None:
        from .bilinear import build_P_bilinear
        build_P_bilinear(self, W)

    def similarity_trainer(self, W0: torch.Tensor, lr: float, batch_size: int = 4):
        from .train import SimilarityTrainer
        return SimilarityTrainer(self, W0, lr, batch_size)

    def set_cosine_mode(self, mode: str) -> None:
        if mode not in ("reference", "per_edge"):
            raise ValueError(f"cosine_mode must be 'reference' or 'per_edge', got {mode!r}")
        if mode != self.cosine_mode:
            self.cosine_mode, self.P_valid = mode, False

    def P_global(self) -> torch.Tensor:
        out = torch.zeros(int(self.local.edge_origin.max()) + 1 if self.E_loc else 0, dtype=self.acc_dtype)
        out[torch.from_numpy(self.local.edge_origin)] = self.P[:self.E_loc].to("cpu")
        return out

    def _bind(self, method: str, *args, **kwargs):
        return self.k.bind(method, *args, **kwargs)

    def _build_plan(self, cur: int, dst: int, tick: int, gamma: float):
        Zold, Znew = self.Zbuf[cur], self.Zbuf[dst]
        per_block = []
        partial_off = self.partial_off
        for i, (b, rows) in enumerate(zip(self.blocks, self.block_rows)):
            steps = []
            ctx = torch.cuda.stream(self.side_streams[i % 2]) if self.side_streams else contextlib.nullcontext()
            with ctx:
                rp, Xb, Zn = self.rowptr[b.local_start:], self.X_loc[self._rows(b)], self._zrows(Znew, b)
                po, lay = partial_off[i], rows.partials
                mir = self.mirrors_p2p[dst][i] if self.p2p else self.mirrors[i]
                steps.append(("event", i, 0))
                if self.d == 0:
                    per_block.append(steps + [("event", i, e) for e in (4, 1, 2, 3)])
                    continue
                T = len(self.tiles)
                cut = (lambda M, t: M) if T == 1 else (lambda M, t: M[:, self.tiles[t][0]:self.tiles[t][1]])
                width = (lambda t: self.d) if T == 1 else (lambda t: self.tiles[t][1] - self.tiles[t][0])
                part = lambda start, t: self.partials[t * partial_off[-1] + po + start:]
                if mir is not None and T > 1:
                    raise AssertionError("column tiles and mirrored launches do not combine")

                def class_launch(items, t):
                    return ("call", self._bind("spmm_update_class", self.colidx, self.P, items.e0, items.len, items.slot,
                                               items.items_per_block, items.rows, items.slot_ptr, b.row0, cut(Zold, t),
                                               cut(Xb, t), gamma, cut(Zn, t), width(t), self.slabs[i % len(self.slabs)],
                                               part(lay.klass, t), mirror=mir, beyond_cache=self.beyond_cache))
                for t in range(T):
                    if rows.owned is not None:
                        steps.append(("call", owned.bind_launch(self, rows.owned.plan, b.row0, cut(Zold, t), cut(Xb, t),
                                                                gamma, cut(Zn, t), width(t), part(lay.klass, t))))
                        if rows.owned.rest is not None:
                            steps.append(class_launch(rows.owned.rest, t))
                    elif rows.klass is not None:
                        steps.append(class_launch(rows.klass, t))
                    if rows.split is not None:
                        steps.append(("call", self._bind("spmm_update_split", rp, self.colidx, self.P, rows.split.rows,
                                                         rows.split.seg_ptr, rows.split.seg_row, self.segment_edges, b.row0,
                                                         cut(Zold, t), cut(Xb, t), gamma, cut(Zn, t), width(t),
                                                         self.slabs[i % len(self.slabs)], part(lay.split, t), mirror=mir)))
                steps.append(("event", i, 4))
                for t in range(T):
                    if rows.hub is not None:
                        steps.append(("call", self._bind("spmm_update_long", rp, self.colidx, self.P, rows.hub, 16,
                                                         b.row0, cut(Zold, t), cut(Xb, t), gamma, cut(Zn, t), width(t),
                                                         part(lay.hub, t), mirror=mir)))
                steps.append(("event", i, 1))
                for t in range(T):
                    if rows.mid is not None:
                        steps.append(("call", self._bind("spmm_update_long", rp, self.colidx, self.P, rows.mid, 4,
                                                         b.row0, cut(Zold, t), cut(Xb, t), gamma, cut(Zn, t), width(t),
                                                         part(lay.mid, t), mirror=mir)))
                steps.append(("event", i, 2))
                for t in range(T):
                    steps.append(("call", self._bind("spmm_update", rp, self.colidx, self.P, b.nrows, b.row0, cut(Zold, t),
                                                     cut(Xb, t), gamma, cut(Zn, t), width(t), self.long_threshold,
                                                     part(lay.main, t), sinks_untouched=True, mirror=mir,
                                                     beyond_cache=self.beyond_cache)))
                steps.append(("event", i, 3))
                if b.span is not None:
                    steps.append(("allgather", Znew[b.span[0]:b.span[1]], Zn))
                elif b.exchange is not None and not self.p2p:
                    ex = b.exchange
                    if self.send_rows[i] is not None and mir is None:
                        steps.append(("call", self._bind("gather_rows", Znew, self.send_rows[i], self.d,
                                                         self.send_buf[i])))
                    steps.append(("alltoall", Znew[ex.recv_start:ex.recv_start + ex.recv_rows], self.send_buf[i],
                                  ex.out_splits, ex.in_splits))
            per_block.append(steps)
        final = self._bind("reduce_partials", self.partials, self.partials.numel(), self.ws,
                           self.delta_pp[tick:tick + 1])
        return per_block, final

    def sweep(self, gamma: float) -> float:
        return self.sweep_wait(self.sweep_launch(gamma))

    def sweep_launch(self, gamma: float) -> int:
        if not self.P_valid:
            raise RuntimeError("sweep() before build_P()")
        stream = torch.cuda.current_stream(self.device).cuda_stream if self.device.type == "cuda" else 0
        src = self.cur
        dst = next(i for i in range(len(self.Zbuf)) if i != src and i != self.hold)
        parity = self._tick
        self._tick ^= 1
        if self._delta_stream is not None and self._delta_busy[parity]:
            torch.cuda.current_stream(self.device).wait_event(self._delta_ev[parity])
            self._delta_busy[parity] = False
        key = (src, dst, parity, float(gamma), stream)
        plan = self._plans.get(key)
        if plan is None:
            plan = self._plans[key] = self._build_plan(src, dst, parity, float(gamma))
        events = None
        if self.time_kernels and len(self.kernel_events) < self.MAX_TIMED_SWEEPS * len(self.blocks):
            events = [[torch.cuda.Event(enable_timing=True) for _ in range(5)] for _ in self.blocks]
            self.kernel_events.extend((i,) + tuple(ev) for i, ev in enumerate(events))
        per_block, final = plan
        works = []
        side = self.side_streams
        if side:
            main = torch.cuda.current_stream(self.device)
            start = torch.cuda.Event()
            start.record(main)
            for st in side:
                st.wait_event(start)
        for i, steps in enumerate(per_block):
            ctx = torch.cuda.stream(side[i % 2]) if side else contextlib.nullcontext()
            with ctx:
# ... 89 lines not shown
```

clane_amd/owned.py:

```python
from __future__ import annotations

from typing import Optional

import numpy as np

from . import xcd
from .blocks import ClassItems, OwnedRows, PartialLayout


def possible(eng) -> bool:
    widths = [c1 - c0 for c0, c1 in eng.tiles]
    return bool(eng.world == 1 and not eng._forced and eng.class_threshold > 0 and eng.d > 0
                and all(eng.k.has_spmm_owned(eng.dtype, w) for w in widths))


def plan_block(eng, layout: PartialLayout, rows_c: np.ndarray, rows_abs: np.ndarray, segments,
               phased: dict) -> Optional[OwnedRows]:
    dev = eng.device
    sizes, seg_len, seg_e0 = segments
    NS = seg_len.size // max(1, sizes.size)
    own = sizes <= eng.owned_max_edges
    if not own.any():
        return None
    n_rest = int((~own).sum())
    pick = lambda a, m: a.reshape(sizes.size, NS)[m].reshape(-1)
    plan = xcd.owned_plan(sizes[own], pick(seg_len, own), pick(seg_e0, own), rows_c[own],
                          layout.owned_slots(n_rest, int(own.sum())), row_edges=eng.owned_row_edges,
                          groups=eng.owned_groups, batch_vrows=eng.owned_batch_vrows)
    eng.owned_balance = plan["group_step_edges"]
    rest = None
    if n_rest:
        keep = ~own
        items = xcd.class_items(eng.local.rowptr, eng.local.colidx, rows_abs[keep], eng.class_chunk, None,
                                row_ids=rows_c[keep], segments=(sizes[keep], pick(seg_len, keep), pick(seg_e0, keep)),
                                **phased)
        rest = ClassItems.upload(items, rows_c[keep], dev)
    return OwnedRows(eng.k.make_owned_plan(plan, eng.owned_chunk, dev), rest, n_rest)


def bind_launch(eng, plan, row0: int, Zold, Xb, gamma: float, Zn, width: int, partials):
    return eng._bind("spmm_update_owned", eng.colidx, eng.P, plan, eng.owned_block_threads, row0, Zold, Xb, gamma, Zn,
                     width, partials, beyond_cache=eng.beyond_cache, loads=eng.owned_loads)
```

clane_amd/xcd.py:

```python
from __future__ import annotations

from typing import Optional

import numpy as np
import torch

XCD_CLASSES = 8


def xcd_class(position):
    p = position
    return (p ^ (p >> 3) ^ (p >> 6) ^ (p >> 9)) & (XCD_CLASSES - 1)


def xcd_subclass(position, row_degree, class_threshold: int, phase_threshold: int = 0, phases: int = 1):
    cls = xcd_class(position)
    if phases > 1 and phase_threshold > 0:
        cls = cls + XCD_CLASSES * (((position >> 6) % phases) * (row_degree > phase_threshold))
    return cls * (row_degree > class_threshold)


CLASS_THRESHOLD_BY_ROWS_PER_WAVE = {1: 64, 2: 64, 4: 256, 8: 256}
CLASS_CHUNK = 256
PHASES_BY_ROWS_PER_WAVE = {1: 4, 2: 2, 4: 1, 8: 1}
# ... 68 lines not shown
        pieces.append((np.zeros(flat, dtype=np.int64), np.zeros(flat, dtype=np.int32),
                       np.full(flat, -1, dtype=np.int32), np.zeros(flat, dtype=np.int32)))
    out_e0, out_len, out_slot, out_row = (np.concatenate([p[i] for p in pieces]) for i in range(4))
    return {"e0": out_e0, "len": out_len, "slot": out_slot, "row": out_row, "slot_ptr": slot_ptr,
            "items_per_block": int(items_per_block)}


def row_segments(rowptr: np.ndarray, colidx: np.ndarray, rows: np.ndarray, colidx_dev: Optional[torch.Tensor] = None,
                 phase_threshold: int = 0, phases: int = 1):
    n = rows.size
    NS = XCD_CLASSES * max(1, phases)
    sizes = (rowptr[rows + 1] - rowptr[rows]).astype(np.int64)
    start = np.concatenate([[0], np.cumsum(sizes)[:-1]])
    if colidx_dev is not None and colidx_dev.is_cuda:
        dev = colidx_dev.device
        seg_len = np.empty(n * NS, dtype=np.int64)
        unsorted = False
        bounds = np.concatenate([[0], np.cumsum(sizes)])
        for a, b in row_pieces(bounds, CLASS_ITEMS_PIECE_EDGES):
            if bounds[b] == bounds[a]:
                seg_len[a * NS:b * NS] = 0
                continue
            sizes_t = torch.from_numpy(sizes[a:b]).to(dev)
            rid = torch.repeat_interleave(torch.arange(b - a, device=dev), sizes_t)
            idx = (torch.from_numpy(rowptr[rows[a:b]] - (start[a:b] - bounds[a])).to(dev)[rid]
                   + torch.arange(int(bounds[b] - bounds[a]), device=dev))
            sub = xcd_subclass(colidx_dev[idx].long(), sizes_t[rid], 0, phase_threshold, phases)
            key = rid * NS + sub
            unsorted = unsorted or (bool((key[1:] < key[:-1]).any()) if key.numel() > 1 else False)
            seg_len[a * NS:b * NS] = torch.bincount(key, minlength=(b - a) * NS).cpu().numpy()
    else:
        idx = np.repeat(rowptr[rows] - start, sizes) + np.arange(int(sizes.sum()), dtype=np.int64)
        rid = np.repeat(np.arange(n, dtype=np.int64), sizes)
        sub = xcd_subclass(colidx[idx].astype(np.int64), sizes[rid], 0, phase_threshold, phases)
        unsorted = idx.size > 1 and bool((np.diff(rid * NS + sub) < 0).any())
        seg_len = np.bincount(rid * NS + sub, minlength=n * NS)
    if unsorted:
        raise AssertionError("class rows must have their edges sorted by (xcd_subclass(column), column)")
    seg_e0 = np.repeat(rowptr[rows], NS) + (np.cumsum(seg_len) - seg_len - np.repeat(start, NS))
    return sizes, seg_len.astype(np.int64), seg_e0


def items_per_block_for(n_items: int) -> int:
    return int(min(CLASS_ITEMS_PER_BLOCK, max(4, 4 * -(-n_items // (4 * 4096)))))


OWNED_MAX_EDGES = 512
OWNED_ROW_EDGES = 1024
OWNED_GROUPS = 256
OWNED_BLOCK_THREADS = 1024
OWNED_LDS_BYTES = 152 * 1024
OWNED_LOADS = 12
OWNED_DEFAULT = True


def owned_plan(sizes: np.ndarray, seg_len: np.ndarray, seg_e0: np.ndarray, row_ids: np.ndarray, row_parts: np.ndarray,
               *, row_edges: int, groups: int, batch_vrows: int) -> Optional[dict]:
    n = int(sizes.size)
    if n == 0:
        return None
    if groups < 1 or row_edges < 64:
        raise ValueError("owned_plan: groups must be >= 1 and row_edges >= 64")
    NS = seg_len.size // n
    seg_len = seg_len.reshape(n, NS).astype(np.int64)
    seg_e0 = seg_e0.reshape(n, NS).astype(np.int64)
    keys = np.nonzero(seg_len.sum(0) > 0)[0]
    if keys.size == 0:
        keys = np.zeros(1, dtype=np.int64)
    S = int(keys.size)
    seg_len, seg_e0 = seg_len[:, keys], seg_e0[:, keys]
    nv = np.maximum(1, -(-sizes // row_edges)).astype(np.int64)
    while True:
        over = (-(-seg_len // nv[:, None])).sum(1) > row_edges
        if not over.any():
            break
        nv[over] += 1
    if int(nv.max()) > batch_vrows:
        raise ValueError(f"owned_plan: a row of {int(nv.max())} virtual rows does not fit a batch of {batch_vrows}")
    row_cum = np.cumsum(seg_len, 1).astype(np.float64)
    share = np.maximum(row_cum.sum(0) / groups, 1.0)
    row_cum /= share
    cum = np.zeros((groups, S))
    group_of = np.empty(n, dtype=np.int64)
    dealt = np.argsort(-sizes, kind="stable")
    for i in dealt.tolist():
        g = int((cum + row_cum[i]).max(1).argmin())
        group_of[i] = g
        cum[g] += row_cum[i]
    order = dealt[np.argsort(group_of[dealt], kind="stable")]
    g_sorted, nv_sorted = group_of[order], nv[order]
    bat_of_row = np.empty(n, dtype=np.int64)
    b, used, g_prev = -1, 0, -1
    for j, (g, k) in enumerate(zip(g_sorted.tolist(), nv_sorted.tolist())):
        if g != g_prev or used + k > batch_vrows:
            b, used, g_prev = b + 1, 0, g
        used += k
        bat_of_row[j] = b
    B = b + 1
    bat_row_ptr = np.zeros(B + 1, dtype=np.int64)
    np.cumsum(np.bincount(bat_of_row, minlength=B), out=bat_row_ptr[1:])
    row_vptr = np.zeros(n + 1, dtype=np.int64)
    np.cumsum(nv_sorted, out=row_vptr[1:])
    bat_vrow_ptr = row_vptr[bat_row_ptr]
    bat_group = g_sorted[bat_row_ptr[:-1]]
    grp_bat_ptr = np.zeros(groups + 1, dtype=np.int64)
    np.cumsum(np.bincount(bat_group, minlength=groups), out=grp_bat_ptr[1:])
# ... 24 lines not shown
```

include/clane_hip.h:

```cpp
#ifndef CLANE_HIP_H_
#define CLANE_HIP_H_

#include <stdint.h>

#ifdef __cplusplus
extern "C" {
#endif

#define CLANE_ABI_VERSION 5

#define CLANE_OK 0
#define CLANE_ERR_INVALID_ARGUMENT (-1)
#define CLANE_ERR_LAUNCH (-2)

#define CLANE_SCORE_REFERENCE 0
#define CLANE_SCORE_PER_EDGE 1
#define CLANE_SCORE_RAW_DOT 2

#define CLANE_SCORE_FUSE_SOFTMAX 1
#define CLANE_SCORE_ROW_PARTS(n) (((n) & 0xff) << 8)

#define CLANE_SPMM_SINKS_UNTOUCHED 1
#define CLANE_SPMM_TABLE_BEYOND_CACHE 2

// ... 88 lines not shown
int clane_spmm_update_split_f64(const int64_t *rowptr, const int32_t *colidx, const double *P,
                                const int32_t *split_rows, const int64_t *seg_ptr, const int32_t *seg_row,
                                int64_t n_split, int64_t n_segments, int64_t edges_per_segment, int64_t row0,
                                const double *Z_old, int64_t ldz, const double *X, int64_t ldx, double gamma,
                                double *Z_new, int64_t ldo, int32_t d, double *slab, const clane_mirror_t *mirror,
                                double *delta_partials, void *stream);
int clane_spmm_update_split_bf16(const int64_t *rowptr, const int32_t *colidx, const float *P,
                                 const int32_t *split_rows, const int64_t *seg_ptr, const int32_t *seg_row,
                                 int64_t n_split, int64_t n_segments, int64_t edges_per_segment, int64_t row0,
                                 const uint16_t *Z_old, int64_t ldz, const uint16_t *X, int64_t ldx, float gamma,
                                 uint16_t *Z_new, int64_t ldo, int32_t d, float *slab, const clane_mirror_t *mirror,
                                 double *delta_partials, void *stream);

int clane_edge_score_class_f32(const int64_t *rowptr, const int32_t *colidx, const int64_t *item_e0,
                               const int32_t *item_len, const int32_t *item_slot, const int32_t *item_row,
                               int64_t n_blocks, int32_t items_per_block, const int32_t *class_rows,
                               const int64_t *slot_ptr, int64_t n_rows, int64_t row0, const float *Z, int64_t ldz,
                               int32_t d, int32_t mode, const double *sums2, const float *sq, float *scores,
                               int32_t flags, float *stats, void *stream);
int clane_edge_score_class_f64(const int64_t *rowptr, const int32_t *colidx, const int64_t *item_e0,
                               const int32_t *item_len, const int32_t *item_slot, const int32_t *item_row,
                               int64_t n_blocks, int32_t items_per_block, const int32_t *class_rows,
                               const int64_t *slot_ptr, int64_t n_rows, int64_t row0, const double *Z, int64_t ldz,
                               int32_t d, int32_t mode, const double *sums2, const double *sq, double *scores,
                               int32_t flags, double *stats, void *stream);
int clane_edge_score_class_bf16(const int64_t *rowptr, const int32_t *colidx, const int64_t *item_e0,
                                const int32_t *item_len, const int32_t *item_slot, const int32_t *item_row,
                                int64_t n_blocks, int32_t items_per_block, const int32_t *class_rows,
                                const int64_t *slot_ptr, int64_t n_rows, int64_t row0, const uint16_t *Z, int64_t ldz,
                                int32_t d, int32_t mode, const double *sums2, const float *sq, float *scores,
                                int32_t flags, float *stats, void *stream);

int64_t clane_spmm_class_slab_len(int64_t n_slots, int32_t d);
int clane_spmm_update_class_f32(const int32_t *colidx, const float *P, const int64_t *item_e0, const int32_t *item_len,
                                const int32_t *item_slot, int64_t n_blocks, int32_t items_per_block,
                                const int32_t *class_rows, const int64_t *slot_ptr, int64_t n_rows, int64_t row0,
                                const float *Z_old, int64_t ldz, const float *X, int64_t ldx, float gamma, float *Z_new,
                                int64_t ldo, int32_t d, int32_t flags, float *slab, const clane_mirror_t *mirror,
                                double *delta_partials, void *stream);
int clane_spmm_update_class_f64(const int32_t *colidx, const double *P, const int64_t *item_e0, const int32_t *item_len,
                                const int32_t *item_slot, int64_t n_blocks, int32_t items_per_block,
                                const int32_t *class_rows, const int64_t *slot_ptr, int64_t n_rows, int64_t row0,
                                const double *Z_old, int64_t ldz, const double *X, int64_t ldx, double gamma,
                                double *Z_new, int64_t ldo, int32_t d, int32_t flags, double *slab, const clane_mirror_t *mirror,
                                double *delta_partials, void *stream);
int clane_spmm_update_class_bf16(const int32_t *colidx, const float *P, const int64_t *item_e0, const int32_t *item_len,
                                 const int32_t *item_slot, int64_t n_blocks, int32_t items_per_block,
                                 const int32_t *class_rows, const int64_t *slot_ptr, int64_t n_rows, int64_t row0,
                                 const uint16_t *Z_old, int64_t ldz, const uint16_t *X, int64_t ldx, float gamma,
                                 uint16_t *Z_new, int64_t ldo, int32_t d, int32_t flags, float *slab, const clane_mirror_t *mirror,
                                 double *delta_partials, void *stream);

#define CLANE_OWNED_LOADS(n) (((n) & 0xff) << 8)
typedef struct {
    const int32_t *grp_bat_ptr;
    const int32_t *bat_vrow_ptr;
    const int32_t *bat_row_ptr;
    const int32_t *bat_seg_ptr;
    const int64_t *seg_e0;
    const int32_t *seg_len;
    const int32_t *seg_vrow;
    const int32_t *row_id;
    const int32_t *row_part;
    const int32_t *row_vptr;
    int32_t n_groups;
    int32_t n_steps;
    int32_t chunk;
    int32_t max_batch_vrows;
} clane_owned_plan_t;
int clane_spmm_update_owned_f32(const int32_t *colidx, const float *P, const clane_owned_plan_t *plan,
                                int32_t block_threads, int64_t row0, const float *Z_old, int64_t ldz, const float *X,
                                int64_t ldx, float gamma, float *Z_new, int64_t ldo, int32_t d, int32_t flags,
                                double *delta_partials, void *stream);

int clane_reduce_partials(const double *partials, int64_t n, double *ws, double *out, void *stream);

int clane_l1_distance_f32(const float *A, int64_t lda, const float *B, int64_t ldb, int64_t nrows, int32_t d,
                          float *sq_a, double *ws, double *out, void *stream);
int clane_l1_distance_f64(const double *A, int64_t lda, const double *B, int64_t ldb, int64_t nrows, int32_t d,
                          double *sq_a, double *ws, double *out, void *stream);
int clane_l1_distance_bf16(const uint16_t *A, int64_t lda, const uint16_t *B, int64_t ldb, int64_t nrows, int32_t d,
                           float *sq_a, double *ws, double *out, void *stream);

int clane_gather_rows_f32(const float *src, int64_t lds, const int32_t *idx, int64_t n, int32_t d, float *dst,
                          int64_t ldd, void *stream);
int clane_gather_rows_f64(const double *src, int64_t lds, const int32_t *idx, int64_t n, int32_t d, double *dst,
                          int64_t ldd, void *stream);
int clane_gather_rows_bf16(const uint16_t *src, int64_t lds, const int32_t *idx, int64_t n, int32_t d, uint16_t *dst,
                           int64_t ldd, void *stream);

int clane_pair_cosine_f32(const float *A, int64_t lda, const float *B, int64_t ldb, int64_t nrows, int32_t d,
                          float *out, double *ws, void *stream);
int clane_pair_cosine_f64(const double *A, int64_t lda, const double *B, int64_t ldb, int64_t nrows, int32_t d,
                          double *out, double *ws, void *stream);

int clane_project_rows_f32(const float *Z, int64_t rows, int32_t d, int64_t ldz, const float *W, float *Y, int64_t ldy,
                           void *stream);
int clane_project_rows_f64(const double *Z, int64_t rows, int32_t d, int64_t ldz, const double *W, double *Y,
                           int64_t ldy, void *stream);
int clane_project_rows_bf16(const uint16_t *Z, int64_t rows, int32_t d, int64_t ldz, const float *W, float *Y,
                            int64_t ldy, void *stream);

int clane_edge_score_pair_f32(const int64_t *rowptr, const int32_t *colidx, int64_t nrows, int64_t row0, const float *S,
                              int64_t lds, const float *N, int64_t ldn, int32_t d, float *scores, int32_t flags,
                              int64_t long_threshold, const int32_t *long_rows, int64_t n_long, void *stream);
int clane_edge_score_pair_f64(const int64_t *rowptr, const int32_t *colidx, int64_t nrows, int64_t row0,
                              const double *S, int64_t lds, const double *N, int64_t ldn, int32_t d, double *scores,
                              int32_t flags, int64_t long_threshold, const int32_t *long_rows, int64_t n_long,
                              void *stream);
int clane_edge_score_class_pair_f32(const int64_t *rowptr, const int32_t *colidx, const int64_t *item_e0,
                                    const int32_t *item_len, const int32_t *item_slot, const int32_t *item_row,
                                    int64_t n_blocks, int32_t items_per_block, const int32_t *class_rows,
                                    const int64_t *slot_ptr, int64_t n_rows, int64_t row0, const float *S, int64_t lds,
                                    const float *N, int64_t ldn, int32_t d, float *scores, int32_t flags, float *stats,
                                    void *stream);
int clane_edge_score_class_pair_f64(const int64_t *rowptr, const int32_t *colidx, const int64_t *item_e0,
                                    const int32_t *item_len, const int32_t *item_slot, const int32_t *item_row,
                                    int64_t n_blocks, int32_t items_per_block, const int32_t *class_rows,
                                    const int64_t *slot_ptr, int64_t n_rows, int64_t row0, const double *S,
                                    int64_t lds, const double *N, int64_t ldn, int32_t d, double *scores,
                                    int32_t flags, double *stats, void *stream);

int clane_pair_project_f32(const float *Z, int64_t table_rows, int32_t d, int64_t ldz, const int32_t *src,
                           const int32_t *dst, int64_t B, const float *W, float *A, float *Bm, void *stream);
int clane_pair_project_f64(const double *Z, int64_t table_rows, int32_t d, int64_t ldz, const int32_t *src,
                           const int32_t *dst, int64_t B, const double *W, double *A, double *Bm, void *stream);
// ... 185 lines not shown
```

Baseline: 283.7 sweeps/s.

## Fuse per-column-tile SpMM update launches into single multi-tile kernels

```diff
diff --git a/clane_amd/_hip.py b/clane_amd/_hip.py
--- a/clane_amd/_hip.py
+++ b/clane_amd/_hip.py
@@ -16,6 +16,7 @@
 SCORE_REFERENCE, SCORE_PER_EDGE, SCORE_RAW_DOT = 0, 1, 2
 SPMM_SINKS_UNTOUCHED = 1
 SPMM_TABLE_BEYOND_CACHE = 2
+OWNED_EPILOGUE_AHEAD = 1 << 16
 SCORE_FUSE_SOFTMAX = 1
 SCORE_MODES = {"reference": SCORE_REFERENCE, "per_edge": SCORE_PER_EDGE, "raw_dot": SCORE_RAW_DOT}
 
@@ -61,6 +62,13 @@
     SIGNATURES[f"clane_l1_distance_{_s}"] = (C.c_int, [_p, _i64, _p, _i64, _i64, _i32, _p, _p, _p, _p])
 SIGNATURES["clane_spmm_update_owned_f32"] = (
     C.c_int, [_p, _p, _p, _i32, _i64, _p, _i64, _p, _i64, C.c_float, _p, _i64, _i32, _i32, _p, _p])
+SIGNATURES["clane_spmm_update_tiles_f32"] = (
+    C.c_int, [_p, _p, _p, _i64, _i64, _p, _i64, _p, _i64, C.c_float, _p, _i64, _i32, _i32, _i64, _i32, _p, _i64, _p])
+SIGNATURES["clane_spmm_update_class_tiles_f32"] = (
+    C.c_int, [_p, _p, _p, _p, _p, _i64, _i32, _p, _p, _i64, _i64, _i64, _p, _i64, _p, _i64, C.c_float, _p, _i64, _i32, _i32,
+              _i32, _p, _p, _i64, _p])
+SIGNATURES["clane_spmm_update_owned_tiles_f32"] = (
+    C.c_int, [_p, _p, _p, _i32, _i64, _p, _i64, _p, _i64, C.c_float, _p, _i64, _i32, _i32, _i32, _p, _i64, _p])
 for _s in ("f32", "f64"):
     SIGNATURES[f"clane_degree_weighted_sums_{_s}"] = (C.c_int, [_p, _p, _p, _i64, _p, _p, _p])
     SIGNATURES[f"clane_edge_score_finalize_{_s}"] = (C.c_int, [_p, _p, _i64, _i64, _i32, _p, _p, _p, _p])
@@ -512,8 +520,28 @@
         raise NotImplementedError(f"{type(self).__name__} has no make_owned_plan")
 
     def spmm_update_owned(self, colidx, P, plan, block_threads: int, row0: int, Z_old, X, gamma: float, Z_new, d: int,
-                          partials, beyond_cache: bool = False, loads: int = 0):
+                          partials, beyond_cache: bool = False, loads: int = 0, ahead: bool = False):
         raise NotImplementedError(f"{type(self).__name__} has no spmm_update_owned")
+
+    def has_spmm_tiles(self, dtype, d: int, tile_cols: int) -> bool:
+        return False
+
+    owned_epilogue_ahead = False
+
+    def spmm_update_tiles(self, rowptr, colidx, P, nrows: int, row0: int, Z_old, X, gamma: float, Z_new, d: int,
+                          tile_cols: int, long_threshold: int, partials, partials_stride: int,
+                          sinks_untouched: bool = False, beyond_cache: bool = False):
+        raise NotImplementedError(f"{type(self).__name__} has no spmm_update_tiles")
+
+    def spmm_update_class_tiles(self, colidx, P, item_e0, item_len, item_slot, items_per_block: int, class_rows, slot_ptr,
+                                n_slots: int, row0: int, Z_old, X, gamma: float, Z_new, d: int, tile_cols: int, slab,
+                                partials, partials_stride: int, beyond_cache: bool = False):
+        raise NotImplementedError(f"{type(self).__name__} has no spmm_update_class_tiles")
+
+    def spmm_update_owned_tiles(self, colidx, P, plan, block_threads: int, row0: int, Z_old, X, gamma: float, Z_new,
+                                d: int, tile_cols: int, partials, partials_stride: int, beyond_cache: bool = False,
+                                loads: int = 0, ahead: bool = False):
+        raise NotImplementedError(f"{type(self).__name__} has no spmm_update_owned_tiles")
 
     def bind(self, method: str, *args, **kwargs):
         fn = getattr(self, method)
@@ -525,6 +553,8 @@
 
 
 class HipKernels(KernelBackend):
+
+    owned_epilogue_ahead = True
 
     def __init__(self, lib: Optional[C.CDLL] = None):
         self.lib = lib if lib is not None else load_library()
@@ -731,7 +761,7 @@
         return OwnedPlan(plan, chunk, device)
 
     def spmm_update_owned(self, colidx, P, plan: OwnedPlan, block_threads: int, row0: int, Z_old, X, gamma: float,
-                          Z_new, d: int, partials, beyond_cache: bool = False, loads: int = 0):
+                          Z_new, d: int, partials, beyond_cache: bool = False, loads: int = 0, ahead: bool = False):
         zo, ldz = _mat(Z_old, "Z_old")
         xp, ldx = _mat(X, "X")
         zn, ldo = _mat(Z_new, "Z_new")
@@ -746,8 +776,78 @@
         self._invoke(self.lib.clane_spmm_update_owned_f32, "clane_spmm_update_owned",
                      _vec(colidx, torch.int32, "colidx"), _vec(P, torch.float32, "P"), C.cast(C.pointer(plan.c), _p),
                      int(block_threads), row0, zo, ldz, xp, ldx, gamma, zn, ldo, d,
-                     (SPMM_TABLE_BEYOND_CACHE if beyond_cache else 0) | ((int(loads) & 0xff) << 8),
+                     (SPMM_TABLE_BEYOND_CACHE if beyond_cache else 0) | ((int(loads) & 0xff) << 8)
+                     | (OWNED_EPILOGUE_AHEAD if ahead else 0),
                      _vec(partials, torch.float64, "partials"), self._stream(Z_old))
+
+    def has_spmm_tiles(self, dtype, d: int, tile_cols: int) -> bool:
+        if dtype != torch.float32 or not 0 < tile_cols <= d or tile_cols % 4:
+            return False
+        lanes = lambda w: next(n for n in (8, 16, 32, 64) if -(-w // 4) <= n or n == 64)
+        return lanes(d - (-(-d // tile_cols) - 1) * tile_cols) == lanes(tile_cols)
+
+    def _tile_args(self, name, Z_old, X, Z_new, d, tile_cols, partials, partials_stride, per_tile):
+        zo, ldz = _mat(Z_old, "Z_old")
+        xp, ldx = _mat(X, "X")
+        zn, ldo = _mat(Z_new, "Z_new")
+        if not (Z_old.dtype == X.dtype == Z_new.dtype == torch.float32):
+            raise TypeError(f"{name}: float32 tables only")
+        if not self.has_spmm_tiles(torch.float32, d, tile_cols) or min(Z_old.shape[1], X.shape[1], Z_new.shape[1]) < d:
+            raise ValueError(f"{name}: no fused launch for d={d} in tiles of {tile_cols} columns")
+        tiles = -(-d // tile_cols)
+        if (tiles > 1 and partials_stride < per_tile) or partials.numel() < (tiles - 1) * partials_stride + per_tile:
+            raise ValueError(f"{name}: the tiles' partials overlap or end outside `partials`")
+        return zo, ldz, xp, ldx, zn, ldo
+
+    def spmm_update_tiles(self, rowptr, colidx, P, nrows: int, row0: int, Z_old, X, gamma: float, Z_new, d: int,
+                          tile_cols: int, long_threshold: int, partials, partials_stride: int,
+                          sinks_untouched: bool = False, beyond_cache: bool = False):
+        zo, ldz, xp, ldx, zn, ldo = self._tile_args("spmm_update_tiles", Z_old, X, Z_new, d, tile_cols, partials,
+                                                    partials_stride, self.spmm_partials_len(nrows, 0))
+        self._invoke(self.lib.clane_spmm_update_tiles_f32, "clane_spmm_update_tiles",
+                     _vec(rowptr, torch.int64, "rowptr"), _vec(colidx, torch.int32, "colidx"), _vec(P, torch.float32, "P"),
+                     nrows, row0, zo, ldz, xp, ldx, gamma, zn, ldo, d, tile_cols, long_threshold,
+                     (SPMM_SINKS_UNTOUCHED if sinks_untouched else 0) | (SPMM_TABLE_BEYOND_CACHE if beyond_cache else 0),
+                     _vec(partials, torch.float64, "partials"), partials_stride, self._stream(Z_old))
+
+    def spmm_update_class_tiles(self, colidx, P, item_e0, item_len, item_slot, items_per_block: int, class_rows, slot_ptr,
+                                n_slots: int, row0: int, Z_old, X, gamma: float, Z_new, d: int, tile_cols: int, slab,
+                                partials, partials_stride: int, beyond_cache: bool = False):
+        zo, ldz, xp, ldx, zn, ldo = self._tile_args("spmm_update_class_tiles", Z_old, X, Z_new, d, tile_cols, partials,
+                                                    partials_stride, class_rows.numel())
+        n_items = item_e0.numel()
+        if n_items % items_per_block or item_len.numel() != n_items or item_slot.numel() != n_items:
+            raise ValueError("spmm_update_class_tiles: the item arrays must hold whole blocks of items_per_block items")
+        if slab.numel() < -(-d // tile_cols) * self.spmm_class_slab_len(n_slots, tile_cols):
+            raise ValueError("spmm_update_class_tiles: the slab does not hold every tile's chunk sums")
+        self._invoke(self.lib.clane_spmm_update_class_tiles_f32, "clane_spmm_update_class_tiles",
+                     _vec(colidx, torch.int32, "colidx"), _vec(P, torch.float32, "P"),
+                     _vec(item_e0, torch.int64, "item_e0"), _vec(item_len, torch.int32, "item_len"),
+                     _vec(item_slot, torch.int32, "item_slot"), n_items // items_per_block, items_per_block,
+                     _vec(class_rows, torch.int32, "class_rows"), _vec(slot_ptr, torch.int64, "slot_ptr"),
+                     class_rows.numel(), n_slots, row0, zo, ldz, xp, ldx, gamma, zn, ldo, d, tile_cols,
+                     SPMM_TABLE_BEYOND_CACHE if beyond_cache else 0, _vec(slab, torch.float32, "slab"),
+                     _vec(partials, torch.float64, "partials"), partials_stride, self._stream(Z_old))
+
+    def spmm_update_owned_tiles(self, colidx, P, plan: OwnedPlan, block_threads: int, row0: int, Z_old, X, gamma: float,
+                                Z_new, d: int, tile_cols: int, partials, partials_stride: int, beyond_cache: bool = False,
+                                loads: int = 0, ahead: bool = False):
+        zo, ldz, xp, ldx, zn, ldo = self._tile_args("spmm_update_owned_tiles", Z_old, X, Z_new, d, tile_cols, partials,
+                                                    partials_stride, plan.max_part + 1)
+        if not self.has_spmm_owned(torch.float32, tile_cols):
+            raise ValueError(f"spmm_update_owned_tiles: no owned instance for tiles of {tile_cols} columns")
+        lanes = 32 if tile_cols <= 128 else 64
+        if plan.max_batch_vrows * lanes * 16 > OWNED_LDS_LIMIT:
+            raise ValueError(f"spmm_update_owned_tiles: {plan.max_batch_vrows} virtual rows per batch do not fit the LDS")
+        if (plan.max_edge > min(colidx.numel(), P.numel()) or plan.max_row >= min(X.shape[0], Z_new.shape[0])
+                or row0 + plan.max_row >= Z_old.shape[0]):
+            raise ValueError("spmm_update_owned_tiles: the plan reaches outside colidx / P or the tables")
+        self._invoke(self.lib.clane_spmm_update_owned_tiles_f32, "clane_spmm_update_owned_tiles",
+                     _vec(colidx, torch.int32, "colidx"), _vec(P, torch.float32, "P"), C.cast(C.pointer(plan.c), _p),
+                     int(block_threads), row0, zo, ldz, xp, ldx, gamma, zn, ldo, d, tile_cols,
+                     (SPMM_TABLE_BEYOND_CACHE if beyond_cache else 0) | ((int(loads) & 0xff) << 8)
+                     | (OWNED_EPILOGUE_AHEAD if ahead else 0),
+                     _vec(partials, torch.float64, "partials"), partials_stride, self._stream(Z_old))
 
     def reduce_partials(self, partials, n: int, ws, out):
         self._invoke(self.lib.clane_reduce_partials, "clane_reduce_partials",
diff --git a/clane_amd/csrc/clane_abi.hip b/clane_amd/csrc/clane_abi.hip
--- a/clane_amd/csrc/clane_abi.hip
+++ b/clane_amd/csrc/clane_abi.hip
@@ -504,12 +504,50 @@
 constexpr int64_t kLdsPerCU = 160 * 1024;
 constexpr int64_t kLdsDefaultLimit = 64 * 1024;
 
+inline int tile_count(int d, int tile_cols) { return int(ceil_div(d, tile_cols)); }
+template <typename T>
+bool tiles_share_layout(int d, int tile_cols) {
+    constexpr int KV = Elem<T>::kVec;
+    auto lanes = [](int w) { const int p = int(ceil_div(w, KV)); return p <= 8 ? 8 : p <= 16 ? 16 : p <= 32 ? 32 : 64; };
+    return tile_cols % KV == 0 && lanes(d - (tile_count(d, tile_cols) - 1) * tile_cols) == lanes(tile_cols);
+}
+
+template <typename T, typename PT>
+int spmm_update_owned_impl(const char *what, const int32_t *colidx, const PT *P, const clane_owned_plan_t *plan,
+                           int32_t block_threads, int64_t row0, const T *Z_old, int64_t ldz, const T *X, int64_t ldx,
+                           typename Elem<T>::acc_t gamma, T *Z_new, int64_t ldo, int32_t d_all, int32_t tile_cols,
+                           int64_t part_stride, int32_t flags, double *delta_partials, void *stream);
+
 template <typename T, typename PT>
 int spmm_update_owned(const int32_t *colidx, const PT *P, const clane_owned_plan_t *plan, int32_t block_threads,
                       int64_t row0, const T *Z_old, int64_t ldz, const T *X, int64_t ldx,
                       typename Elem<T>::acc_t gamma, T *Z_new, int64_t ldo, int32_t d, int32_t flags,
                       double *delta_partials, void *stream) {
+    return spmm_update_owned_impl<T, PT>("spmm_update_owned", colidx, P, plan, block_threads, row0, Z_old, ldz, X, ldx,
+                                         gamma, Z_new, ldo, d, d, 0, flags, delta_partials, stream);
+}
+
+template <typename T, typename PT>
+int spmm_update_owned_tiles(const int32_t *colidx, const PT *P, const clane_owned_plan_t *plan, int32_t block_threads,
+                            int64_t row0, const T *Z_old, int64_t ldz, const T *X, int64_t ldx,
+                            typename Elem<T>::acc_t gamma, T *Z_new, int64_t ldo, int32_t d, int32_t tile_cols,
+                            int32_t flags, double *delta_partials, int64_t partials_tile_stride, void *stream) {
+    REQUIRE(d > 0 && tile_cols > 0 && tile_cols <= d && partials_tile_stride >= 0 && tiles_share_layout<T>(d, tile_cols),
+            "spmm_update_owned_tiles: tile_cols must be a multiple of the 16-byte pack in (0, d] whose last tile keeps the "
+            "lane layout, the partials' stride >= 0 (d=%d tile_cols=%d)", d, tile_cols);
+    return spmm_update_owned_impl<T, PT>("spmm_update_owned_tiles", colidx, P, plan, block_threads, row0, Z_old, ldz, X,
+                                         ldx, gamma, Z_new, ldo, d, tile_cols, partials_tile_stride, flags, delta_partials,
+                                         stream);
+}
+
+template <typename T, typename PT>
+int spmm_update_owned_impl(const char *what, const int32_t *colidx, const PT *P, const clane_owned_plan_t *plan,
+                           int32_t block_threads, int64_t row0, const T *Z_old, int64_t ldz, const T *X, int64_t ldx,
+                           typename Elem<T>::acc_t gamma, T *Z_new, int64_t ldo, int32_t d_all, int32_t tile_cols,
+                           int64_t part_stride, int32_t flags, double *delta_partials, void *stream) {
     using A = typename Elem<T>::acc_t;
+    const int32_t d = tile_cols;
+    REQUIRE(d_all >= d, "%s: bad shape", what);
     REQUIRE(plan, "spmm_update_owned: null plan");
     REQUIRE(plan->n_groups >= 0 && row0 >= 0 && d > 0, "spmm_update_owned: bad shape");
     REQUIRE(plan->n_steps >= 1 && plan->n_steps <= kOwnedMaxSteps, "spmm_update_owned: n_steps must be in [1, %d]",
@@ -517,7 +555,7 @@
     REQUIRE(plan->chunk >= kWave && plan->chunk % kWave == 0, "spmm_update_owned: chunk must be a positive multiple of 64");
     REQUIRE(block_threads >= kWave && block_threads <= kOwnedMaxBlock && block_threads % kWave == 0,
             "spmm_update_owned: block_threads must be a multiple of 64 in [64, %d]", kOwnedMaxBlock);
-    REQUIRE(ldz >= d && ldx >= d && ldo >= d, "spmm_update_owned: leading dimension < d");
+    REQUIRE(ldz >= d_all && ldx >= d_all && ldo >= d_all, "spmm_update_owned: leading dimension < d");
     REQUIRE(plan->max_batch_vrows >= 0, "spmm_update_owned: negative max_batch_vrows");
     if (plan->n_groups == 0) return CLANE_OK;
     REQUIRE(colidx && P && plan->grp_bat_ptr && plan->bat_vrow_ptr && plan->bat_row_ptr && plan->bat_seg_ptr &&
@@ -552,7 +590,7 @@
             }
         }
         kernel<<<unsigned(plan->n_groups), unsigned(block_threads), size_t(lds), (hipStream_t)stream>>>(
-            colidx, P, op, row0, Z_old, ldz, X, ldx, gamma, Z_new, ldo, d, beyond, delta_partials);
+            colidx, P, op, row0, Z_old, ldz, X, ldx, gamma, Z_new, ldo, d_all, tile_cols, part_stride, (flags & CLANE_OWNED_EPILOGUE_AHEAD) != 0, beyond, delta_partials);
     };
     constexpr int KV = Elem<T>::kVec;
     const int asked = (flags >> 8) & 0xff;
@@ -568,7 +606,111 @@
         else launch.template operator()<KV, 64, 8>();
     }
     if (rc != CLANE_OK) return rc;
-    return check_launch("spmm_update_owned");
+    return check_launch(what);
+}
+
+template <typename T, typename PT>
+int spmm_update_tiles(const int64_t *rowptr, const int32_t *colidx, const PT *P, int64_t nrows, int64_t row0,
+                      const T *Z_old, int64_t ldz, const T *X, int64_t ldx, typename Elem<T>::acc_t gamma, T *Z_new,
+                      int64_t ldo, int32_t d, int32_t tile_cols, int64_t long_threshold, int32_t flags,
+                      double *delta_partials, int64_t partials_tile_stride, void *stream) {
+    REQUIRE(nrows >= 0 && row0 >= 0 && d > 0, "spmm_update_tiles: bad shape nrows=%lld row0=%lld d=%d", (long long)nrows,
+            (long long)row0, d);
+    REQUIRE(tile_cols > 0 && tile_cols <= d && tiles_share_layout<T>(d, tile_cols),
+            "spmm_update_tiles: tile_cols must be a multiple of the 16-byte pack in (0, d] whose last tile keeps the lane "
+            "layout (d=%d tile_cols=%d)", d, tile_cols);
+    REQUIRE(ldz >= d && ldx >= d && ldo >= d, "spmm_update_tiles: leading dimension < d");
+    REQUIRE(long_threshold >= 0, "spmm_update_tiles: negative long_threshold");
+    REQUIRE(delta_partials, "spmm_update_tiles: null delta_partials");
+    const int n_tiles = tile_count(d, tile_cols);
+    const int per_tile = int(spmm_main_grid(nrows));
+    REQUIRE(partials_tile_stride >= (n_tiles > 1 ? per_tile : 0), "spmm_update_tiles: the tiles' partials overlap");
+    REQUIRE(int64_t(n_tiles) * per_tile <= INT32_MAX, "spmm_update_tiles: grid too large");
+    if (nrows == 0) return CLANE_OK;
+    REQUIRE(rowptr && colidx && P && Z_old && X && Z_new, "spmm_update_tiles: null pointer");
+    REQUIRE((const void *)Z_new != (const void *)Z_old, "spmm_update_tiles: Z_new must not alias Z_old (Jacobi sweep)");
+    const Layout L = pick_layout<T>(tile_cols, {Z_old, X, Z_new}, {ldz, ldx, ldo});
+    REQUIRE(L.vec, "spmm_update_tiles: the tables must allow 16-byte packs");
+    const TileGrid tg{per_tile, tile_cols, partials_tile_stride};
+    const unsigned grid = unsigned(n_tiles) * unsigned(per_tile);
+    const bool sinks = (flags & CLANE_SPMM_SINKS_UNTOUCHED) != 0, beyond = (flags & CLANE_SPMM_TABLE_BEYOND_CACHE) != 0;
+    dispatch_layout<T>(L, [&]<int VEC, int LPR>() {
+        if constexpr (VEC > 1) {
+            constexpr int U = CLANE_SPMM_U;
+            if constexpr (LPR == 32 && VEC == 4 && sizeof(T) == 4) {
+                if (beyond) {
+                    spmm_update_subrow_tiles_kernel<T, PT, VEC, LPR, CLANE_SUBROW_U32><<<grid, kBlock, 0, (hipStream_t)stream>>>(
+                        rowptr, colidx, P, nrows, row0, Z_old, ldz, X, ldx, gamma, Z_new, ldo, d, long_threshold, sinks,
+                        rows_per_block(nrows), beyond, tg, delta_partials);
+                    return;
+                }
+            }
+            if constexpr (LPR < kWave)
+                spmm_update_subrow_tiles_kernel<T, PT, VEC, LPR, U><<<grid, kBlock, 0, (hipStream_t)stream>>>(
+                    rowptr, colidx, P, nrows, row0, Z_old, ldz, X, ldx, gamma, Z_new, ldo, d, long_threshold, sinks,
+                    rows_per_block(nrows), beyond, tg, delta_partials);
+            else
+                spmm_update_tiles_kernel<T, PT, VEC, LPR, U><<<grid, kBlock, 0, (hipStream_t)stream>>>(
+                    rowptr, colidx, P, nrows, row0, Z_old, ldz, X, ldx, gamma, Z_new, ldo, d, long_threshold, sinks,
+                    rows_per_block(nrows), beyond, tg, delta_partials);
+        }
+    });
+    return check_launch("spmm_update_tiles");
+}
+
+template <typename T, typename PT>
+int spmm_update_class_tiles(const int32_t *colidx, const PT *P, const int64_t *item_e0, const int32_t *item_len,
+                            const int32_t *item_slot, int64_t n_blocks, int32_t items_per_block,
+                            const int32_t *class_rows, const int64_t *slot_ptr, int64_t n_rows, int64_t n_slots,
+                            int64_t row0, const T *Z_old, int64_t ldz, const T *X, int64_t ldx,
+                            typename Elem<T>::acc_t gamma, T *Z_new, int64_t ldo, int32_t d, int32_t tile_cols,
+                            int32_t flags, typename Elem<T>::acc_t *slab, double *delta_partials,
+                            int64_t partials_tile_stride, void *stream) {
+    REQUIRE(n_blocks >= 0 && n_blocks <= INT32_MAX - 8 && n_rows >= 0 && n_rows <= INT32_MAX && n_slots >= 0 && row0 >= 0 &&
+                d > 0, "spmm_update_class_tiles: bad shape");
+    REQUIRE(tile_cols > 0 && tile_cols <= d && tiles_share_layout<T>(d, tile_cols),
+            "spmm_update_class_tiles: tile_cols must be a multiple of the 16-byte pack in (0, d] whose last tile keeps the "
+            "lane layout (d=%d tile_cols=%d)", d, tile_cols);
+    REQUIRE(items_per_block >= kWavesPerBlock && items_per_block <= kMaxItemsPerBlock,
+            "spmm_update_class_tiles: items_per_block must be in [%d, %d]", kWavesPerBlock, kMaxItemsPerBlock);
+    REQUIRE(ldz >= d && ldx >= d && ldo >= d, "spmm_update_class_tiles: leading dimension < d");
+    const int n_tiles = tile_count(d, tile_cols);
+    REQUIRE(partials_tile_stride >= (n_tiles > 1 ? n_rows : 0), "spmm_update_class_tiles: the tiles' partials overlap");
+    if (n_rows == 0) return CLANE_OK;
+    REQUIRE(colidx && P && item_e0 && item_len && item_slot && class_rows && slot_ptr && Z_old && X && Z_new && slab &&
+                delta_partials, "spmm_update_class_tiles: null pointer");
+    REQUIRE((const void *)Z_new != (const void *)Z_old, "spmm_update_class_tiles: Z_new must not alias Z_old");
+    REQUIRE(aligned16(slab), "spmm_update_class_tiles: slab must be 16-byte aligned");
+    const Layout L = pick_layout<T>(tile_cols, {Z_old, X, Z_new}, {ldz, ldx, ldo});
+    REQUIRE(L.vec, "spmm_update_class_tiles: the tables must allow 16-byte packs");
+    const int64_t ld_slab = ceil_div(tile_cols, 8) * 8;
+    const int64_t slab_stride = n_slots * ld_slab;
+    const int chunk_blocks = int(ceil_div(n_blocks, 8) * 8);
+    const bool beyond = (flags & CLANE_SPMM_TABLE_BEYOND_CACHE) != 0;
+    REQUIRE(int64_t(n_tiles) * chunk_blocks <= INT32_MAX, "spmm_update_class_tiles: grid too large");
+    dispatch_layout<T>(L, [&]<int VEC, int LPR>() {
+        if constexpr (VEC > 1) {
+            constexpr int U = CLANE_LONG_U;
+            constexpr int kDeepU = (LPR == 32 && VEC == 4 && sizeof(T) == 4) ? CLANE_CLASS_U32 : 0;
+            const TileGrid cg{chunk_blocks, tile_cols, 0};
+            const unsigned grid = unsigned(n_tiles) * unsigned(chunk_blocks);
+            if (n_blocks > 0 && kDeepU > 0 && beyond)
+                spmm_class_chunk_tiles_kernel<T, PT, VEC, LPR, (kDeepU > 0 ? kDeepU : U)>
+                    <<<grid, kBlock, 0, (hipStream_t)stream>>>(colidx, P, item_e0, item_len, item_slot, int(n_blocks),
+                                                               items_per_block, Z_old, ldz, d, slab, ld_slab, slab_stride, cg);
+            else if (n_blocks > 0)
+                spmm_class_chunk_tiles_kernel<T, PT, VEC, LPR, U><<<grid, kBlock, 0, (hipStream_t)stream>>>(
+                    colidx, P, item_e0, item_len, item_slot, int(n_blocks), items_per_block, Z_old, ldz, d, slab, ld_slab,
+                    slab_stride, cg);
+            const int combine_blocks = int(ceil_div(n_rows, kWave / LPR));
+            const TileGrid bg{combine_blocks, tile_cols, partials_tile_stride};
+            spmm_class_combine_tiles_kernel<T, VEC, LPR>
+                <<<unsigned(n_tiles) * unsigned(combine_blocks), kCombineWaves * kWave, 0, (hipStream_t)stream>>>(
+                    class_rows, slot_ptr, n_rows, row0, slab, ld_slab, slab_stride, Z_old, ldz, X, ldx, gamma, Z_new, ldo, d,
+                    beyond, bg, delta_partials);
+        }
+    });
+    return check_launch("spmm_update_class_tiles");
 }
 
 template <typename T>
@@ -1363,6 +1505,33 @@
     return spmm_update_owned<float, float>(colidx, P, plan, block_threads, row0, Z_old, ldz, X, ldx, gamma, Z_new, ldo,
                                            d, flags, delta_partials, stream);
 }
+int clane_spmm_update_tiles_f32(const int64_t *rowptr, const int32_t *colidx, const float *P, int64_t nrows, int64_t row0,
+                                const float *Z_old, int64_t ldz, const float *X, int64_t ldx, float gamma, float *Z_new,
+                                int64_t ldo, int32_t d, int32_t tile_cols, int64_t long_threshold, int32_t flags,
+                                double *delta_partials, int64_t partials_tile_stride, void *stream) {
+    return spmm_update_tiles<float, float>(rowptr, colidx, P, nrows, row0, Z_old, ldz, X, ldx, gamma, Z_new, ldo, d,
+                                           tile_cols, long_threshold, flags, delta_partials, partials_tile_stride, stream);
+}
+int clane_spmm_update_class_tiles_f32(const int32_t *colidx, const float *P, const int64_t *item_e0,
+                                      const int32_t *item_len, const int32_t *item_slot, int64_t n_blocks,
+                                      int32_t items_per_block, const int32_t *class_rows, const int64_t *slot_ptr,
+                                      int64_t n_rows, int64_t n_slots, int64_t row0, const float *Z_old, int64_t ldz,
+                                      const float *X, int64_t ldx, float gamma, float *Z_new, int64_t ldo, int32_t d,
+                                      int32_t tile_cols, int32_t flags, float *slab, double *delta_partials,
+                                      int64_t partials_tile_stride, void *stream) {
+    return spmm_update_class_tiles<float, float>(colidx, P, item_e0, item_len, item_slot, n_blocks, items_per_block,
+                                                 class_rows, slot_ptr, n_rows, n_slots, row0, Z_old, ldz, X, ldx, gamma,
+                                                 Z_new, ldo, d, tile_cols, flags, slab, delta_partials,
+                                                 partials_tile_stride, stream);
+}
+int clane_spmm_update_owned_tiles_f32(const int32_t *colidx, const float *P, const clane_owned_plan_t *plan,
+                                      int32_t block_threads, int64_t row0, const float *Z_old, int64_t ldz,
+                                      const float *X, int64_t ldx, float gamma, float *Z_new, int64_t ldo, int32_t d,
+                                      int32_t tile_cols, int32_t flags, double *delta_partials,
+                                      int64_t partials_tile_stride, void *stream) {
+    return spmm_update_owned_tiles<float, float>(colidx, P, plan, block_threads, row0, Z_old, ldz, X, ldx, gamma, Z_new,
+                                                 ldo, d, tile_cols, flags, delta_partials, partials_tile_stride, stream);
+}
 int64_t clane_spmm_class_slab_len(int64_t n_slots, int32_t d) { return n_slots * (ceil_div(d, 8) * 8); }
 int64_t clane_spmm_split_slab_len(int64_t n_segments, int32_t d) { return n_segments * (ceil_div(d, 8) * 8); }
 
diff --git a/clane_amd/csrc/spmm_update.h b/clane_amd/csrc/spmm_update.h
--- a/clane_amd/csrc/spmm_update.h
+++ b/clane_amd/csrc/spmm_update.h
@@ -190,11 +190,11 @@
 #endif
 
 template <typename T, typename PT, int VEC, int LPR, int U, bool MIRRORED>
-__global__ CLANE_SPMM_BOUNDS void spmm_update_kernel(
+__device__ __forceinline__ void spmm_update_block(
     const int64_t *__restrict__ rowptr, const int32_t *__restrict__ colidx, const PT *__restrict__ P, int64_t nrows,
     int64_t row0, const T *__restrict__ Zold, int64_t ldz, const T *__restrict__ X, int64_t ldx,
     typename Elem<T>::acc_t gamma, T *__restrict__ Znew, int64_t ldo, int d, int64_t long_threshold,
-    bool skip_sinks, int rows_per_block, Mirror<T> mirror, bool nt_store, double *__restrict__ partials) {
+    bool skip_sinks, int rows_per_block, Mirror<T> mirror, bool nt_store, int64_t block, double *__restrict__ partial) {
     using A = typename Elem<T>::acc_t;
     __shared__ int64_t s_rowptr[kMaxRowsPerBlock + 1];
     __shared__ int64_t s_mptr[MIRRORED ? kMaxRowsPerBlock + 1 : 1];
@@ -206,7 +206,7 @@
     const int wave = __builtin_amdgcn_readfirstlane(threadIdx.x / kWave);
     const int sub = lane / LPR;
     const int sl = lane % LPR;
-    const int64_t row_begin = int64_t(blockIdx.x) * rows_per_block;
+    const int64_t row_begin = block * rows_per_block;
     const int nb = int((row_begin + rows_per_block < nrows ? row_begin + rows_per_block : nrows) - row_begin);
 
     for (int i = threadIdx.x; i <= nb; i += kBlock) {
@@ -303,7 +303,43 @@
     double dsum = 0.0;
     for (int i = lane; i < nb; i += kWave) dsum += s_rowsum[i];
     dsum = group_sum<kWave>(dsum);
-    if (lane == 0) partials[blockIdx.x] = dsum;
+    if (lane == 0) *partial = dsum;
+}
+
+template <typename T, typename PT, int VEC, int LPR, int U, bool MIRRORED>
+__global__ CLANE_SPMM_BOUNDS void spmm_update_kernel(
+    const int64_t *__restrict__ rowptr, const int32_t *__restrict__ colidx, const PT *__restrict__ P, int64_t nrows,
+    int64_t row0, const T *__restrict__ Zold, int64_t ldz, const T *__restrict__ X, int64_t ldx,
+    typename Elem<T>::acc_t gamma, T *__restrict__ Znew, int64_t ldo, int d, int64_t long_threshold,
+    bool skip_sinks, int rows_per_block, Mirror<T> mirror, bool nt_store, double *__restrict__ partials) {
+    spmm_update_block<T, PT, VEC, LPR, U, MIRRORED>(rowptr, colidx, P, nrows, row0, Zold, ldz, X, ldx, gamma, Znew, ldo, d,
+                                                    long_threshold, skip_sinks, rows_per_block, mirror, nt_store,
+                                                    blockIdx.x, partials + blockIdx.x);
+}
+
+struct TileGrid {
+    int per_tile;
+    int tile_cols;
+    int64_t part_stride;
+    __device__ __forceinline__ int tile() const { return int(blockIdx.x) / per_tile; }
+    __device__ __forceinline__ int width(int tile, int d) const {
+        return d - tile * tile_cols < tile_cols ? d - tile * tile_cols : tile_cols;
+    }
+};
+
+template <typename T, typename PT, int VEC, int LPR, int U>
+__global__ CLANE_SPMM_BOUNDS void spmm_update_tiles_kernel(
+    const int64_t *__restrict__ rowptr, const int32_t *__restrict__ colidx, const PT *__restrict__ P, int64_t nrows,
+    int64_t row0, const T *__restrict__ Zold, int64_t ldz, const T *__restrict__ X, int64_t ldx,
+    typename Elem<T>::acc_t gamma, T *__restrict__ Znew, int64_t ldo, int d, int64_t long_threshold,
+    bool skip_sinks, int rows_per_block, bool nt_store, TileGrid tg, double *__restrict__ partials) {
+    const int tile = tg.tile();
+    const int block = int(blockIdx.x) - tile * tg.per_tile;
+    const int c = tile * tg.tile_cols;
+    spmm_update_block<T, PT, VEC, LPR, U, false>(rowptr, colidx, P, nrows, row0, Zold + c, ldz, X + c, ldx, gamma,
+                                                 Znew + c, ldo, tg.width(tile, d), long_threshold, skip_sinks,
+                                                 rows_per_block, Mirror<T>{nullptr, nullptr, nullptr, 0}, nt_store, block,
+                                                 partials + tile * tg.part_stride + block);
 }
 
 #ifndef CLANE_SUBROW_MIN_WAVES
@@ -315,11 +351,11 @@
 #define CLANE_SUBROW_BOUNDS __launch_bounds__(kBlock)
 #endif
 template <typename T, typename PT, int VEC, int LPR, int U, bool MIRRORED>
-__global__ CLANE_SUBROW_BOUNDS void spmm_update_subrow_kernel(
+__device__ __forceinline__ void spmm_update_subrow_block(
     const int64_t *__restrict__ rowptr, const int32_t *__restrict__ colidx, const PT *__restrict__ P, int64_t nrows,
     int64_t row0, const T *__restrict__ Zold, int64_t ldz, const T *__restrict__ X, int64_t ldx,
     typename Elem<T>::acc_t gamma, T *__restrict__ Znew, int64_t ldo, int d, int64_t long_threshold,
-    bool skip_sinks, int rows_per_block, Mirror<T> mirror, bool nt_store, double *__restrict__ partials) {
+    bool skip_sinks, int rows_per_block, Mirror<T> mirror, bool nt_store, int64_t block, double *__restrict__ partial) {
     using A = typename Elem<T>::acc_t;
     static_assert(LPR < kWave, "use spmm_update_kernel for rows that fill a wave");
     static_assert(LPR % U == 0, "a sub-wave's edge buffer is consumed in whole groups of U");
@@ -333,7 +369,7 @@
     const int sub = lane / LPR;
     const int sl = lane % LPR;
     const int sub_base = sub * LPR;
-    const int64_t row_begin = int64_t(blockIdx.x) * rows_per_block;
+    const int64_t row_begin = block * rows_per_block;
     const int nb = int((row_begin + rows_per_block < nrows ? row_begin + rows_per_block : nrows) - row_begin);
     const int c0 = sl * VEC;
     const bool col_ok = c0 < d;
@@ -452,7 +488,33 @@
     double dsum = 0.0;
     for (int i = lane; i < nb; i += kWave) dsum += s_rowsum[i];
     dsum = group_sum<kWave>(dsum);
-    if (lane == 0) partials[blockIdx.x] = dsum;
+    if (lane == 0) *partial = dsum;
+}
+
+template <typename T, typename PT, int VEC, int LPR, int U, bool MIRRORED>
+__global__ CLANE_SUBROW_BOUNDS void spmm_update_subrow_kernel(
+    const int64_t *__restrict__ rowptr, const int32_t *__restrict__ colidx, const PT *__restrict__ P, int64_t nrows,
+    int64_t row0, const T *__restrict__ Zold, int64_t ldz, const T *__restrict__ X, int64_t ldx,
+    typename Elem<T>::acc_t gamma, T *__restrict__ Znew, int64_t ldo, int d, int64_t long_threshold,
+    bool skip_sinks, int rows_per_block, Mirror<T> mirror, bool nt_store, double *__restrict__ partials) {
+    spmm_update_subrow_block<T, PT, VEC, LPR, U, MIRRORED>(rowptr, colidx, P, nrows, row0, Zold, ldz, X, ldx, gamma, Znew,
+                                                           ldo, d, long_threshold, skip_sinks, rows_per_block, mirror,
+                                                           nt_store, blockIdx.x, partials + blockIdx.x);
+}
+
+template <typename T, typename PT, int VEC, int LPR, int U>
+__global__ CLANE_SUBROW_BOUNDS void spmm_update_subrow_tiles_kernel(
+    const int64_t *__restrict__ rowptr, const int32_t *__restrict__ colidx, const PT *__restrict__ P, int64_t nrows,
+    int64_t row0, const T *__restrict__ Zold, int64_t ldz, const T *__restrict__ X, int64_t ldx,
+    typename Elem<T>::acc_t gamma, T *__restrict__ Znew, int64_t ldo, int d, int64_t long_threshold,
+    bool skip_sinks, int rows_per_block, bool nt_store, TileGrid tg, double *__restrict__ partials) {
+    const int tile = tg.tile();
+    const int block = int(blockIdx.x) - tile * tg.per_tile;
+    const int c = tile * tg.tile_cols;
+    spmm_update_subrow_block<T, PT, VEC, LPR, U, false>(rowptr, colidx, P, nrows, row0, Zold + c, ldz, X + c, ldx, gamma,
+                                                        Znew + c, ldo, tg.width(tile, d), long_threshold, skip_sinks,
+                                                        rows_per_block, Mirror<T>{nullptr, nullptr, nullptr, 0}, nt_store,
+                                                        block, partials + tile * tg.part_stride + block);
 }
 
 template <typename T, typename PT, int VEC, int LPR, int U, int WAVES>
@@ -601,10 +663,11 @@
 }
 
 template <typename T, typename PT, int VEC, int LPR, int U>
-__global__ __launch_bounds__(kBlock) void spmm_class_chunk_kernel(
+__device__ __forceinline__ void spmm_class_chunk_block(
     const int32_t *__restrict__ colidx, const PT *__restrict__ P, const int64_t *__restrict__ item_e0,
     const int32_t *__restrict__ item_len, const int32_t *__restrict__ item_slot, int items_per_block,
-    const T *__restrict__ Zold, int64_t ldz, int d, typename Elem<T>::acc_t *__restrict__ slab, int64_t ld_slab) {
+    const T *__restrict__ Zold, int64_t ldz, int d, typename Elem<T>::acc_t *__restrict__ slab, int64_t ld_slab,
+    int64_t block) {
     using A = typename Elem<T>::acc_t;
     __shared__ int64_t s_e0[kMaxItemsPerBlock];
     __shared__ int s_len[kMaxItemsPerBlock];
@@ -614,7 +677,7 @@
     const int wave = __builtin_amdgcn_readfirstlane(threadIdx.x / kWave);
     const int sub = lane / LPR;
     const int sl = lane % LPR;
-    const int64_t base = int64_t(blockIdx.x) * items_per_block;
+    const int64_t base = block * items_per_block;
     for (int i = threadIdx.x; i < items_per_block; i += kBlock) {
         s_e0[i] = item_e0[base + i];
         s_len[i] = item_len[base + i];
@@ -670,6 +733,29 @@
     }
 }
 
+template <typename T, typename PT, int VEC, int LPR, int U>
+__global__ __launch_bounds__(kBlock) void spmm_class_chunk_kernel(
+    const int32_t *__restrict__ colidx, const PT *__restrict__ P, const int64_t *__restrict__ item_e0,
+    const int32_t *__restrict__ item_len, const int32_t *__restrict__ item_slot, int items_per_block,
+    const T *__restrict__ Zold, int64_t ldz, int d, typename Elem<T>::acc_t *__restrict__ slab, int64_t ld_slab) {
+    spmm_class_chunk_block<T, PT, VEC, LPR, U>(colidx, P, item_e0, item_len, item_slot, items_per_block, Zold, ldz, d,
+                                               slab, ld_slab, blockIdx.x);
+}
+
+template <typename T, typename PT, int VEC, int LPR, int U>
+__global__ __launch_bounds__(kBlock) void spmm_class_chunk_tiles_kernel(
+    const int32_t *__restrict__ colidx, const PT *__restrict__ P, const int64_t *__restrict__ item_e0,
+    const int32_t *__restrict__ item_len, const int32_t *__restrict__ item_slot, int n_blocks, int items_per_block,
+    const T *__restrict__ Zold, int64_t ldz, int d, typename Elem<T>::acc_t *__restrict__ slab, int64_t ld_slab,
+    int64_t slab_stride, TileGrid tg) {
+    const int tile = tg.tile();
+    const int block = int(blockIdx.x) - tile * tg.per_tile;
+    if (block >= n_blocks) return;
+    spmm_class_chunk_block<T, PT, VEC, LPR, U>(colidx, P, item_e0, item_len, item_slot, items_per_block,
+                                               Zold + tile * tg.tile_cols, ldz, tg.width(tile, d),
+                                               slab + tile * slab_stride, ld_slab, block);
+}
+
 constexpr int kCombineWaves = CLANE_COMBINE_WAVES;
 #ifndef CLANE_COMBINE_LOADS
 #define CLANE_COMBINE_LOADS 16
@@ -677,18 +763,18 @@
 constexpr int kCombineLoads = CLANE_COMBINE_LOADS;
 
 template <typename T, int VEC, int LPR>
-__global__ __launch_bounds__(kCombineWaves *kWave) void spmm_class_combine_kernel(
+__device__ __forceinline__ void spmm_class_combine_block(
     const int32_t *__restrict__ class_rows, const int64_t *__restrict__ slot_ptr, int64_t n_rows, int64_t row0,
     const typename Elem<T>::acc_t *__restrict__ slab, int64_t ld_slab, const T *__restrict__ Zold, int64_t ldz,
     const T *__restrict__ X, int64_t ldx, typename Elem<T>::acc_t gamma, T *__restrict__ Znew, int64_t ldo, int d,
-    Mirror<T> mirror, bool nt_store, double *__restrict__ partials) {
+    Mirror<T> mirror, bool nt_store, int64_t block, double *__restrict__ partials) {
     using A = typename Elem<T>::acc_t;
     constexpr int kRows = kWave / LPR;
     __shared__ A s_part[kCombineWaves > 1 ? kCombineWaves - 1 : 1][kWave][VEC];
     const int lane = lane_id();
     const int wave = __builtin_amdgcn_readfirstlane(threadIdx.x / kWave);
     const int sub = lane / LPR, sl = lane % LPR;
-    const int64_t i = int64_t(blockIdx.x) * kRows + sub;
+    const int64_t i = block * kRows + sub;
     const bool live = i < n_rows;
     const int64_t r = live ? class_rows[i] : 0;
     const int64_t s0 = live ? slot_ptr[i] : 0, s1 = live ? slot_ptr[i + 1] : 0;
@@ -750,6 +836,31 @@
         rsum = group_sum<LPR>(rsum);
         if (live && sl == 0) partials[i] = double(rsum);
     }
+}
+
+template <typename T, int VEC, int LPR>
+__global__ __launch_bounds__(kCombineWaves *kWave) void spmm_class_combine_kernel(
+    const int32_t *__restrict__ class_rows, const int64_t *__restrict__ slot_ptr, int64_t n_rows, int64_t row0,
+    const typename Elem<T>::acc_t *__restrict__ slab, int64_t ld_slab, const T *__restrict__ Zold, int64_t ldz,
+    const T *__restrict__ X, int64_t ldx, typename Elem<T>::acc_t gamma, T *__restrict__ Znew, int64_t ldo, int d,
+    Mirror<T> mirror, bool nt_store, double *__restrict__ partials) {
+    spmm_class_combine_block<T, VEC, LPR>(class_rows, slot_ptr, n_rows, row0, slab, ld_slab, Zold, ldz, X, ldx, gamma,
+                                          Znew, ldo, d, mirror, nt_store, blockIdx.x, partials);
+}
+
+template <typename T, int VEC, int LPR>
+__global__ __launch_bounds__(kCombineWaves *kWave) void spmm_class_combine_tiles_kernel(
+    const int32_t *__restrict__ class_rows, const int64_t *__restrict__ slot_ptr, int64_t n_rows, int64_t row0,
+    const typename Elem<T>::acc_t *__restrict__ slab, int64_t ld_slab, int64_t slab_stride, const T *__restrict__ Zold,
+    int64_t ldz, const T *__restrict__ X, int64_t ldx, typename Elem<T>::acc_t gamma, T *__restrict__ Znew, int64_t ldo,
+    int d, bool nt_store, TileGrid tg, double *__restrict__ partials) {
+    const int tile = tg.tile();
+    const int block = int(blockIdx.x) - tile * tg.per_tile;
+    const int c = tile * tg.tile_cols;
+    spmm_class_combine_block<T, VEC, LPR>(class_rows, slot_ptr, n_rows, row0, slab + tile * slab_stride, ld_slab, Zold + c,
+                                          ldz, X + c, ldx, gamma, Znew + c, ldo, tg.width(tile, d),
+                                          Mirror<T>{nullptr, nullptr, nullptr, 0}, nt_store, block,
+                                          partials + tile * tg.part_stride);
 }
 
 constexpr int kOwnedMaxSteps = 64;
@@ -774,7 +885,8 @@
 __global__ __launch_bounds__(kOwnedMaxBlock) void spmm_owned_kernel(
     const int32_t *__restrict__ colidx, const PT *__restrict__ P, OwnedPlan plan, int64_t row0,
     const T *__restrict__ Zold, int64_t ldz, const T *__restrict__ X, int64_t ldx, typename Elem<T>::acc_t gamma,
-    T *__restrict__ Znew, int64_t ldo, int d, bool nt_store, double *__restrict__ partials) {
+    T *__restrict__ Znew, int64_t ldo, int d_left, int tile_cols, int64_t part_stride, bool ahead, bool nt_store,
+    double *__restrict__ partials) {
     using A = typename Elem<T>::acc_t;
     constexpr int W = LPR * VEC;
     constexpr int kRows = kWave / LPR;
@@ -787,12 +899,14 @@
     const int nwaves = int(blockDim.x) / kWave;
     const int sub = lane / LPR, sl = lane % LPR;
     const int c0 = sl * VEC;
-    const bool col_ok = c0 < d;
-    const T *zcol = Zold + (col_ok ? c0 : 0);
     const int n_steps = plan.n_steps;
     const int64_t chunk = plan.chunk;
     const int b0 = plan.grp_bat_ptr[blockIdx.x], b1 = plan.grp_bat_ptr[blockIdx.x + 1];
 
+    for (; d_left > 0; d_left -= tile_cols, Zold += tile_cols, X += tile_cols, Znew += tile_cols, partials += part_stride) {
+    const int d = d_left < tile_cols ? d_left : tile_cols;
+    const bool col_ok = c0 < d;
+    const T *zcol = Zold + (col_ok ? c0 : 0);
     for (int b = b0; b < b1; ++b) {
         const int v0 = plan.bat_vrow_ptr[b];
         const int nv = plan.bat_vrow_ptr[b + 1] - v0;
@@ -853,6 +967,60 @@
         }
         const int r0 = plan.bat_row_ptr[b];
         const int nr = plan.bat_row_ptr[b + 1] - r0;
+        if (ahead) {
+            struct RowIds {
+                int r, va, vb, part;
+                bool live;
+            };
+            const int stride = nwaves * kRows;
+            auto ids_of = [&](int j0) -> RowIds {
+                RowIds m{0, 0, 0, 0, false};
+                const int j = j0 + sub;
+                if (j0 < nr && j < nr) {
+                    m.r = plan.row_id[r0 + j];
+                    m.va = plan.row_vptr[r0 + j] - v0;
+                    m.vb = plan.row_vptr[r0 + j + 1] - v0;
+                    m.part = plan.row_part[r0 + j];
+                    m.live = true;
+                }
+                return m;
+            };
+            auto request = [&](const RowIds &m, Pack<T, VEC> &x, Pack<T, VEC> &zo) {
+                if (m.live && col_ok) {
+                    x = load_pack_stream<T, VEC>(X + int64_t(m.r) * ldx + c0);
+                    zo = load_pack_stream<T, VEC>(Zold + (row0 + m.r) * ldz + c0);
+                }
+            };
+            int j0 = wave * kRows;
+            RowIds cur = ids_of(j0), nxt = ids_of(j0 + stride);
+            Pack<T, VEC> x{}, zo{};
+            request(cur, x, zo);
+            for (; j0 < nr; j0 += stride) {
+                const RowIds far = ids_of(j0 + 2 * stride);
+                Pack<T, VEC> xn{}, zon{};
+                request(nxt, xn, zon);
+                A rsum = A(0);
+                if (cur.live && col_ok) {
+                    A acc[VEC];
+                    const Pack<A, VEC> first = load_pack<A, VEC>(s_sum + cur.va * W + c0);
+#pragma unroll
+                    for (int k = 0; k < VEC; ++k) acc[k] = first.v[k];
+                    for (int v = cur.va + 1; v < cur.vb; ++v) {
+                        const Pack<A, VEC> t = load_pack<A, VEC>(s_sum + v * W + c0);
+#pragma unroll
+                        for (int k = 0; k < VEC; ++k) acc[k] += t.v[k];
+                    }
+                    Pack<T, VEC> out{};
+                    rsum = finish_pack<T, VEC>(x, zo, acc, gamma, true, Znew + int64_t(cur.r) * ldo + c0, out, nt_store);
+                }
+                rsum = group_sum<LPR>(rsum);
+                if (cur.live && sl == 0) partials[cur.part] = double(rsum);
+                cur = nxt;
+                nxt = far;
+                x = xn;
+                zo = zon;
+            }
+        } else
         for (int j0 = wave * kRows; j0 < nr; j0 += nwaves * kRows) {
             const int j = j0 + sub;
             const bool live = j < nr;
@@ -880,6 +1048,7 @@
         }
         __syncthreads();
     }
-}
-
-}
+    }
+}
+
+}
diff --git a/clane_amd/diagnostics.py b/clane_amd/diagnostics.py
--- a/clane_amd/diagnostics.py
+++ b/clane_amd/diagnostics.py
@@ -37,11 +37,12 @@
                 "hub": int(per_row[is_hub].sum()), "split": int(per_row[is_split | is_class].sum())}
 
     def launches_per_sweep(self) -> int:
-        return len(self.blocks) * len(self.tiles)
+        return len(self.blocks) * (1 if getattr(self, "fused_tiles", None) else len(self.tiles))
 
     def kernel_names(self):
         narrow = self.d > 0 and lanes_per_row(self.d_plan if len(self.tiles) > 1 else self.d, self.dtype) < 64
-        return {"main": "spmm_update_subrow_kernel" if narrow else "spmm_update_kernel",
+        fused = getattr(self, "fused_tiles", frozenset())
+        return {"main": ("spmm_update_subrow" if narrow else "spmm_update") + ("_tiles_kernel" if "row" in fused else "_kernel"),
                 "mid": "spmm_long_kernel<4 waves>", "hub": "spmm_long_kernel<16 waves>",
                 "split": ("spmm_owned_kernel+spmm_class_chunk_kernel+combine" if getattr(self, "class_owned", False)
                           else "spmm_class_chunk_kernel+combine") if self.class_threshold > 0
@@ -74,6 +75,9 @@
                                     "batch_vrows": self.owned_batch_vrows, "chunk": self.owned_chunk,
                                     "loads": self.owned_loads}}
                    if getattr(self, "class_owned", False) else {}),
+                **({"fused_tiles": sorted(self.fused_tiles)} if getattr(self, "fused_tiles", None) else {}),
+                **({"owned_ahead": True} if getattr(self, "class_owned", False) and getattr(self, "owned_ahead", False)
+                   else {}),
                 }
 
     def exchange_bytes_per_sweep(self) -> int:
diff --git a/clane_amd/engine.py b/clane_amd/engine.py
--- a/clane_amd/engine.py
+++ b/clane_amd/engine.py
@@ -8,7 +8,7 @@
 import numpy as np
 import torch
 
-from . import _hip, owned, xcd
+from . import _hip, fused, owned, xcd
 from .blocks import BlockRows, ClassItems, PartialLayout, SplitRows
 from .comm import TorchComm
 from .diagnostics import DiagnosticsMixin
@@ -40,7 +40,7 @@
                  owned_max_edges: int = xcd.OWNED_MAX_EDGES, owned_row_edges: int = xcd.OWNED_ROW_EDGES,
                  owned_groups: int = xcd.OWNED_GROUPS, owned_lds_bytes: int = xcd.OWNED_LDS_BYTES,
                  owned_block_threads: int = xcd.OWNED_BLOCK_THREADS, owned_chunk: Optional[int] = None,
-                 owned_loads: int = xcd.OWNED_LOADS):
+                 owned_loads: int = xcd.OWNED_LOADS, owned_ahead: Optional[bool] = None, fused_tiles=None):
         if X.dim() != 2 or X.shape[0] != csr.num_vertices:
             raise ValueError(f"X must be [V, d] with V={csr.num_vertices}, got {tuple(X.shape)}")
         if cosine_mode not in ("reference", "per_edge"):
@@ -62,6 +62,9 @@
         self._choose_owned(class_owned, owned_max_edges, owned_row_edges, owned_groups, owned_lds_bytes,
                            owned_block_threads, owned_chunk)
         self.owned_loads = int(owned_loads)
+        ahead = xcd.OWNED_EPILOGUE_AHEAD if owned_ahead is None else bool(owned_ahead)
+        self.owned_ahead = bool(ahead and self.k.owned_epilogue_ahead)
+        self._choose_fused_tiles(fused_tiles)
         self._build_layout(csr, chunks, shuffle, seed, hot_rows_first)
         self._choose_row_bins(long_threshold, hub_threshold)
         deg = self._upload_structure()
@@ -166,6 +169,32 @@
         self.owned_chunk = int(chunk) if chunk is not None else self.class_chunk
         if self.class_owned:
             self._check_owned_settings()
+
+    FUSED_PASSES = ("row", "class", "owned")
+
+    def _choose_fused_tiles(self, asked) -> None:
+        w = self.tiles[0][1] - self.tiles[0][0]
+        uniform = all(c0 == t * w and c1 == c0 + w for t, (c0, c1) in enumerate(self.tiles))
+        self.fused_possible = bool(len(self.tiles) > 1 and uniform and self.world == 1 and not self._forced
+                                   and self.dtype == torch.float32
+                                   and fused.backend_has(self, w))
+        if asked is None:
+            want = xcd.FUSED_TILES_DEFAULT
+        elif isinstance(asked, bool):
+            want = self.FUSED_PASSES if asked else ()
+        else:
+            want = tuple(asked)
+            if any(p not in self.FUSED_PASSES for p in want):
+                raise ValueError(f"fused_tiles: passes are {self.FUSED_PASSES}, got {asked!r}")
+        self.fused_tiles = frozenset(want) if self.fused_possible else frozenset()
+
+    def set_fused_tiles(self, on, ahead: Optional[bool] = None) -> None:
+        if self.device.type == "cuda":
+            torch.cuda.synchronize(self.device)
+        self._choose_fused_tiles(on)
+        if ahead is not None:
+            self.owned_ahead = bool(ahead and self.k.owned_epilogue_ahead)
+        self._plans = {}
 
     def _check_owned_settings(self) -> None:
         widths = [c1 - c0 for c0, c1 in self.tiles]
@@ -289,7 +318,8 @@
         self.partials = torch.zeros(self.partial_off[-1] * len(self.tiles), dtype=torch.float64, device=dev)
         slab_len = max(1, self.k.spmm_split_slab_len(max_segments, max(self.d_plan, 1)))
         if max_slots:
-            slab_len = max(slab_len, self.k.spmm_class_slab_len(max_slots, max(self.d_plan, 1)), 2 * max_slots)
+            slab_len = max(slab_len, (len(self.tiles) if self.fused_possible else 1)
+                           * self.k.spmm_class_slab_len(max_slots, max(self.d_plan, 1)), 2 * max_slots)
         self.slabs = [torch.zeros(slab_len, dtype=self.acc_dtype, device=dev)
                       for _ in range(2 if len(self.blocks) > 1 else 1)]
 
@@ -634,19 +664,30 @@
                 if mir is not None and T > 1:
                     raise AssertionError("column tiles and mirrored launches do not combine")
 
+                on = self.fused_tiles if (T > 1 and mir is None) else frozenset()
+                tile_cols, stride, slab = width(0), partial_off[-1], self.slabs[i % len(self.slabs)]
+
+                def class_launch_tiles(items):
+                    return ("call", fused.bind_class(self, items, b.row0, Zold, Xb, gamma, Zn, tile_cols, slab,
+                                                     part(lay.klass, 0), stride))
+
                 def class_launch(items, t):
                     return ("call", self._bind("spmm_update_class", self.colidx, self.P, items.e0, items.len, items.slot,
                                                items.items_per_block, items.rows, items.slot_ptr, b.row0, cut(Zold, t),
                                                cut(Xb, t), gamma, cut(Zn, t), width(t), self.slabs[i % len(self.slabs)],
                                                part(lay.klass, t), mirror=mir, beyond_cache=self.beyond_cache))
+                if rows.owned is not None and "owned" in on:
+                    steps.append(("call", owned.bind_launch_tiles(self, rows.owned.plan, b.row0, Zold, Xb, gamma, Zn,
+                                                                  tile_cols, part(lay.klass, 0), stride)))
+                klass = rows.klass if rows.owned is None else rows.owned.rest
+                if klass is not None and "class" in on:
+                    steps.append(class_launch_tiles(klass))
                 for t in range(T):
-                    if rows.owned is not None:
+                    if rows.owned is not None and "owned" not in on:
                         steps.append(("call", owned.bind_launch(self, rows.owned.plan, b.row0, cut(Zold, t), cut(Xb, t),
                                                                 gamma, cut(Zn, t), width(t), part(lay.klass, t))))
-                        if rows.owned.rest is not None:
-                            steps.append(class_launch(rows.owned.rest, t))
-                    elif rows.klass is not None:
-                        steps.append(class_launch(rows.klass, t))
+                    if klass is not None and "class" not in on:
+                        steps.append(class_launch(klass, t))
                     if rows.split is not None:
                         steps.append(("call", self._bind("spmm_update_split", rp, self.colidx, self.P, rows.split.rows,
                                                          rows.split.seg_ptr, rows.split.seg_row, self.segment_edges, b.row0,
@@ -665,7 +706,10 @@
                                                          b.row0, cut(Zold, t), cut(Xb, t), gamma, cut(Zn, t), width(t),
                                                          part(lay.mid, t), mirror=mir)))
                 steps.append(("event", i, 2))
-                for t in range(T):
+                if "row" in on:
+                    steps.append(("call", fused.bind_row(self, rp, b.nrows, b.row0, Zold, Xb, gamma, Zn, tile_cols,
+                                                         part(lay.main, 0), stride)))
+                for t in range(T if "row" not in on else 0):
                     steps.append(("call", self._bind("spmm_update", rp, self.colidx, self.P, b.nrows, b.row0, cut(Zold, t),
                                                      cut(Xb, t), gamma, cut(Zn, t), width(t), self.long_threshold,
                                                      part(lay.main, t), sinks_untouched=True, mirror=mir,
diff --git a/clane_amd/fused.py b/clane_amd/fused.py
--- /dev/null
+++ b/clane_amd/fused.py
@@ -0,0 +1,16 @@
+from __future__ import annotations
+
+
+def backend_has(eng, tile_cols: int) -> bool:
+    return bool(eng.k.has_spmm_tiles(eng.dtype, eng.d, tile_cols))
+
+
+def bind_row(eng, rowptr, nrows: int, row0: int, Zold, Xb, gamma: float, Zn, tile_cols: int, partials, stride: int):
+    return eng._bind("spmm_update_tiles", rowptr, eng.colidx, eng.P, nrows, row0, Zold, Xb, gamma, Zn, eng.d, tile_cols,
+                     eng.long_threshold, partials, stride, sinks_untouched=True, beyond_cache=eng.beyond_cache)
+
+
+def bind_class(eng, items, row0: int, Zold, Xb, gamma: float, Zn, tile_cols: int, slab, partials, stride: int):
+    return eng._bind("spmm_update_class_tiles", eng.colidx, eng.P, items.e0, items.len, items.slot, items.items_per_block,
+                     items.rows, items.slot_ptr, int(items.slot_ptr[-1]), row0, Zold, Xb, gamma, Zn, eng.d, tile_cols,
+                     slab, partials, stride, beyond_cache=eng.beyond_cache)
diff --git a/clane_amd/owned.py b/clane_amd/owned.py
--- a/clane_amd/owned.py
+++ b/clane_amd/owned.py
@@ -40,4 +40,14 @@
 
 def bind_launch(eng, plan, row0: int, Zold, Xb, gamma: float, Zn, width: int, partials):
     return eng._bind("spmm_update_owned", eng.colidx, eng.P, plan, eng.owned_block_threads, row0, Zold, Xb, gamma, Zn,
-                     width, partials, beyond_cache=eng.beyond_cache, loads=eng.owned_loads)
+                     width, partials, beyond_cache=eng.beyond_cache, loads=eng.owned_loads, **_ahead(eng))
+
+
+def _ahead(eng) -> dict:
+    return {"ahead": True} if getattr(eng, "owned_ahead", False) else {}
+
+
+def bind_launch_tiles(eng, plan, row0: int, Zold, Xb, gamma: float, Zn, tile_cols: int, partials, stride: int):
+    return eng._bind("spmm_update_owned_tiles", eng.colidx, eng.P, plan, eng.owned_block_threads, row0, Zold, Xb, gamma,
+                     Zn, eng.d, tile_cols, partials, stride, beyond_cache=eng.beyond_cache, loads=eng.owned_loads,
+                     **_ahead(eng))
diff --git a/clane_amd/xcd.py b/clane_amd/xcd.py
--- a/clane_amd/xcd.py
+++ b/clane_amd/xcd.py
@@ -144,6 +144,8 @@
 OWNED_LDS_BYTES = 152 * 1024
 OWNED_LOADS = 12
 OWNED_DEFAULT = True
+FUSED_TILES_DEFAULT = ("row", "class", "owned")
+OWNED_EPILOGUE_AHEAD = True
 
 
 def owned_plan(sizes: np.ndarray, seg_len: np.ndarray, seg_e0: np.ndarray, row_ids: np.ndarray, row_parts: np.ndarray,
diff --git a/include/clane_hip.h b/include/clane_hip.h
--- a/include/clane_hip.h
+++ b/include/clane_hip.h
@@ -164,6 +164,7 @@
                                  double *delta_partials, void *stream);
 
 #define CLANE_OWNED_LOADS(n) (((n) & 0xff) << 8)
+#define CLANE_OWNED_EPILOGUE_AHEAD (1 << 16)
 typedef struct {
     const int32_t *grp_bat_ptr;
     const int32_t *bat_vrow_ptr;
@@ -184,6 +185,23 @@
                                 int32_t block_threads, int64_t row0, const float *Z_old, int64_t ldz, const float *X,
                                 int64_t ldx, float gamma, float *Z_new, int64_t ldo, int32_t d, int32_t flags,
                                 double *delta_partials, void *stream);
+
+int clane_spmm_update_tiles_f32(const int64_t *rowptr, const int32_t *colidx, const float *P, int64_t nrows, int64_t row0,
+                                const float *Z_old, int64_t ldz, const float *X, int64_t ldx, float gamma, float *Z_new,
+                                int64_t ldo, int32_t d, int32_t tile_cols, int64_t long_threshold, int32_t flags,
+                                double *delta_partials, int64_t partials_tile_stride, void *stream);
+int clane_spmm_update_class_tiles_f32(const int32_t *colidx, const float *P, const int64_t *item_e0,
+                                      const int32_t *item_len, const int32_t *item_slot, int64_t n_blocks,
+                                      int32_t items_per_block, const int32_t *class_rows, const int64_t *slot_ptr,
+                                      int64_t n_rows, int64_t n_slots, int64_t row0, const float *Z_old, int64_t ldz,
+                                      const float *X, int64_t ldx, float gamma, float *Z_new, int64_t ldo, int32_t d,
+                                      int32_t tile_cols, int32_t flags, float *slab, double *delta_partials,
+                                      int64_t partials_tile_stride, void *stream);
+int clane_spmm_update_owned_tiles_f32(const int32_t *colidx, const float *P, const clane_owned_plan_t *plan,
+                                      int32_t block_threads, int64_t row0, const float *Z_old, int64_t ldz,
+                                      const float *X, int64_t ldx, float gamma, float *Z_new, int64_t ldo, int32_t d,
+                                      int32_t tile_cols, int32_t flags, double *delta_partials,
+                                      int64_t partials_tile_stride, void *stream);
 
 int clane_reduce_partials(const double *partials, int64_t n, double *ws, double *out, void *stream);
 
```

After: 286.8 sweeps/s (median of 6 runs). 1.01x the previous value.
